# madsjulia/GeostatInversion.jl

Measured on AMD Instinct MI355X. Metric: randSVD GB/s + top-k singular-value rel-err, n=1e6 rank=256, higher is better.
Workload: dtype f64

## Files before the change

### geostatinversion.jl_amd/_lib.py

```python
import ctypes as C
import os

import numpy as np

_HERE = os.path.dirname(os.path.abspath(__file__))
LIB_PATH = os.path.join(_HERE, "libgsi_hip.so")

GSI_OK = 0
ERR_NAMES = {1: "GSI_ERR_ARG", 2: "GSI_ERR_NEG_ITERS", 3: "GSI_ERR_SINGULAR", 4: "GSI_ERR_HIP",
             5: "GSI_ERR_RCCL", 6: "GSI_ERR_OOM", 7: "GSI_ERR_NOT_POSDEF", 8: "GSI_ERR_INTERNAL"}
PHASES = ["gemm_n", "gemm_t", "lu", "qr", "svd", "small_gemm", "comm", "other", "comm_wait"]
UNIQUE_ID_BYTES = 128

c_i64 = C.c_int64
c_dp = C.POINTER(C.c_double)
c_vp = C.c_void_p
RANDN_FN = C.CFUNCTYPE(None, c_vp, c_dp, c_i64)

SIGNATURES = {
    "gsi_version": (C.c_int, []),
    "gsi_last_error": (C.c_char_p, []),
    "gsi_backend_name": (C.c_char_p, []),
    "gsi_ctx_create": (C.c_int, [C.POINTER(c_vp), C.c_int]),
    "gsi_ctx_destroy": (C.c_int, [c_vp]),
    "gsi_ctx_sync": (C.c_int, [c_vp]),
    "gsi_comm_unique_id": (C.c_int, [c_vp]),
    "gsi_ctx_comm_init": (C.c_int, [c_vp, C.c_int, C.c_int, c_vp]),
    "gsi_ctx_rank": (C.c_int, [c_vp, C.POINTER(C.c_int), C.POINTER(C.c_int)]),
    "gsi_ctx_host_allgather": (C.c_int, [c_vp, c_dp, c_i64, c_dp]),
    "gsi_op_dense": (C.c_int, [c_vp, C.POINTER(c_vp), c_dp, c_i64, c_i64, c_i64, c_i64, c_i64]),
    "gsi_op_lowrank": (C.c_int, [c_vp, C.POINTER(c_vp), c_dp, c_i64, c_i64, c_i64, C.c_int, c_i64, c_i64]),
    "gsi_op_lowrank_synthetic": (C.c_int, [c_vp, C.POINTER(c_vp), c_i64, c_i64, C.c_uint64, C.c_double, c_i64, c_i64]),
    "gsi_op_lowrank_samples": (C.c_int, [c_vp, c_vp, c_dp, c_i64]),
    "gsi_fftrf_fields": (C.c_int, [c_vp, c_vp, C.c_int, C.POINTER(c_i64), C.c_double, C.c_double, C.c_double, c_dp, c_i64,
                                   C.c_uint64, c_i64]),
    "gsi_op_lowrank_fftrf": (C.c_int, [c_vp, C.POINTER(c_vp), C.c_int, C.POINTER(c_i64), C.c_double, C.c_double, C.c_double,
                                       c_i64, C.c_uint64, c_i64, c_i64]),
    "gsi_fftrf_interpolate": (C.c_int, [c_vp, c_vp, c_vp, C.c_int, C.POINTER(c_i64), c_dp, c_i64, c_dp, c_i64]),
    "gsi_fftrf_spread": (C.c_int, [c_vp, c_vp, c_vp, C.c_int, C.POINTER(c_i64), c_dp, c_i64, c_dp, c_i64]),
    "gsi_fftrf_fields_at": (C.c_int, [c_vp, c_vp, C.c_int, C.POINTER(c_i64), C.c_double, C.c_double, C.c_double, c_dp, c_i64,
                                      C.c_uint64, c_i64, c_dp, c_i64, c_dp, c_i64]),
    "gsi_op_lowrank_fftrf_at": (C.c_int, [c_vp, C.POINTER(c_vp), C.c_int, C.POINTER(c_i64), C.c_double, C.c_double, C.c_double,
                                          c_i64, C.c_uint64, c_dp, c_i64, c_dp, c_i64, c_i64]),
    "gsi_op_dense_gridcov": (C.c_int, [c_vp, C.POINTER(c_vp), c_i64, c_i64, C.c_double, C.c_int, c_i64, c_i64]),
    "gsi_op_gridcov_implicit": (C.c_int, [c_vp, C.POINTER(c_vp), c_i64, c_i64, C.c_double, c_i64, c_i64]),
    "gsi_op_gridcov_implicit_kind": (C.c_int, [c_vp, C.POINTER(c_vp), c_i64, c_i64, C.c_double, C.c_int, c_i64, c_i64]),
    "gsi_op_gridcov_implicit_table": (C.c_int, [c_vp, C.POINTER(c_vp), c_i64, c_i64, c_dp, c_i64, c_i64]),
    "gsi_op_pointcov_implicit": (C.c_int, [c_vp, C.POINTER(c_vp), c_dp, c_i64, C.c_int, C.c_int, C.c_double, C.c_double,
                                           C.c_double, c_i64, c_i64]),
    "gsi_op_fft_powerlaw": (C.c_int, [c_vp, C.POINTER(c_vp), C.c_int, C.POINTER(c_i64), C.c_double]),
    "gsi_op_fft_powerlaw_fftrf": (C.c_int, [c_vp, C.POINTER(c_vp), C.c_int, C.POINTER(c_i64), C.c_double]),
    "gsi_op_fft_gridcov": (C.c_int, [c_vp, C.POINTER(c_vp), C.c_int, C.POINTER(c_i64), C.c_int, c_dp, C.c_double, C.c_double,
                                     C.c_double]),
    "gsi_op_fft_gridcov_table": (C.c_int, [c_vp, C.POINTER(c_vp), C.c_int, C.POINTER(c_i64), c_dp, c_dp, C.c_double]),
    "gsi_op_fft_at": (C.c_int, [c_vp, C.POINTER(c_vp), c_vp, c_dp, c_i64, c_dp]),
    "gsi_gridcov_sampler_create": (C.c_int, [c_vp, C.POINTER(c_vp), C.c_int, C.POINTER(c_i64), C.POINTER(c_i64), C.c_int, c_dp,
                                             C.c_double, C.c_double, C.c_double, C.c_double, c_dp]),
    "gsi_gridcov_sampler_info": (C.c_int, [c_vp, C.POINTER(c_i64), c_dp]),
    "gsi_gridcov_sampler_spectrum": (C.c_int, [c_vp, c_vp, c_dp]),
    "gsi_gridcov_sampler_destroy": (C.c_int, [c_vp]),
    "gsi_gridcov_fields": (C.c_int, [c_vp, c_vp, c_vp, c_dp, c_i64, C.c_uint64, c_i64]),
    "gsi_op_lowrank_gridcov": (C.c_int, [c_vp, C.POINTER(c_vp), c_vp, c_i64, C.c_uint64, c_i64, c_i64]),
    "gsi_op_destroy": (C.c_int, [c_vp]),
    "gsi_op_size": (C.c_int, [c_vp, C.POINTER(c_i64), C.POINTER(c_i64), C.POINTER(c_i64), C.POINTER(c_i64)]),
    "gsi_op_mul": (C.c_int, [c_vp, c_vp, C.c_int, c_dp, c_i64, c_i64, c_dp, c_i64]),
    "gsi_rangefinder": (C.c_int, [c_vp, c_vp, c_dp, c_i64, c_i64, c_dp]),
    "gsi_randsvd": (C.c_int, [c_vp, c_vp, c_dp, c_i64, c_i64, c_i64, c_dp, c_dp]),
    "gsi_randsvd_dense_host": (C.c_int, [c_vp, c_dp, c_i64, c_i64, c_i64, c_dp, c_i64, c_i64, c_i64, c_dp, c_dp, C.POINTER(c_vp)]),
    "gsi_rangefinder_dense_host": (C.c_int, [c_vp, c_dp, c_i64, c_i64, c_i64, c_dp, c_i64, c_i64, c_dp, C.POINTER(c_vp)]),
    "gsi_eig_nystrom": (C.c_int, [c_vp, c_vp, c_dp, c_i64, c_dp, c_dp]),
    "gsi_rangefinder_adaptive": (C.c_int, [c_vp, c_vp, RANDN_FN, c_vp, C.c_double, c_i64, c_dp, C.POINTER(c_i64)]),
    "gsi_mat_create": (C.c_int, [c_vp, C.POINTER(c_vp), c_i64, c_i64]),
    "gsi_mat_destroy": (C.c_int, [c_vp]),
    "gsi_mat_upload": (C.c_int, [c_vp, c_vp, c_dp, c_i64]),
    "gsi_mat_download": (C.c_int, [c_vp, c_vp, c_dp, c_i64]),
    "gsi_mat_randn": (C.c_int, [c_vp, c_vp, C.c_uint64]),
    "gsi_op_mul_dev": (C.c_int, [c_vp, c_vp, C.c_int, c_vp, c_vp]),
    "gsi_rangefinder_dev": (C.c_int, [c_vp, c_vp, c_vp, c_i64, c_vp]),
    "gsi_randsvd_dev": (C.c_int, [c_vp, c_vp, c_vp, c_i64, c_i64, c_i64, c_vp, c_vp]),
    "gsi_randsvd_rows": (C.c_int, [c_vp, c_vp, c_vp, c_i64, c_i64, c_i64, c_vp, c_vp]),
    "gsi_lu_L": (C.c_int, [c_vp, c_dp, c_i64, c_i64, c_dp, C.POINTER(C.c_int32)]),
    "gsi_lu_L_dev": (C.c_int, [c_vp, c_vp, C.POINTER(C.c_int32)]),
    "gsi_lu_L_sharded": (C.c_int, [c_vp, c_dp, c_i64, c_i64, c_dp, C.POINTER(C.c_int32)]),
    "gsi_lu_L_sharded_virtual": (C.c_int, [c_vp, c_dp, c_i64, c_i64, C.c_int, c_dp, C.POINTER(C.c_int32)]),
    "gsi_qr_thinQ": (C.c_int, [c_vp, c_dp, c_i64, c_i64, c_dp, c_dp]),
    "gsi_svd_tall": (C.c_int, [c_vp, c_dp, c_i64, c_i64, c_dp, c_dp]),
    "gsi_gemm": (C.c_int, [c_vp, C.c_int, c_i64, c_i64, c_i64, C.c_double, c_dp, c_i64, c_dp, c_i64, c_dp, c_i64]),
    "gsi_gemm_view": (C.c_int, [c_vp, C.c_int, C.c_int, c_i64, c_i64, c_i64, C.c_double, C.c_double, c_dp, c_i64, c_i64,
                                c_dp, c_i64, c_i64, c_dp, c_i64, c_i64, c_i64, c_i64, C.POINTER(c_i64)]),
    "gsi_cq_gram_round": (C.c_int, [c_vp, c_i64, C.c_int, c_dp, c_dp, c_dp, C.POINTER(C.c_int32), C.POINTER(C.c_int32),
                                    C.POINTER(C.c_double)]),
    "gsi_pcga_params": (C.c_int, [c_vp, c_dp, c_i64, c_i64, c_dp, c_dp, C.c_double, c_dp]),
    "gsi_pcga_update": (C.c_int, [c_vp, c_dp, c_i64, c_i64, c_dp, C.c_double, c_dp, c_i64, c_dp, c_dp]),
    "gsi_pcga_params_dev": (C.c_int, [c_vp, c_vp, c_i64, c_dp, c_dp, C.c_double, c_dp]),
    "gsi_pcga_update_dev": (C.c_int, [c_vp, c_vp, c_i64, c_dp, C.c_double, c_dp, c_i64, c_dp, c_dp]),
    "gsi_mat_download_col": (C.c_int, [c_vp, c_vp, c_i64, c_dp]),
    "gsi_op_lowrank_solve": (C.c_int, [c_vp, c_vp, c_dp, c_dp, C.POINTER(c_i64)]),
    "gsi_op_solve_cg": (C.c_int, [c_vp, c_vp, c_dp, c_vp, c_vp, C.c_double, c_i64, C.POINTER(c_i64), c_dp, C.POINTER(c_i64)]),
    "gsi_op_solve": (C.c_int, [c_vp, c_vp, c_dp, c_dp, c_i64, c_i64, c_dp, c_i64, C.c_double, c_i64, C.POINTER(c_i64), c_dp,
                               C.POINTER(c_i64)]),
    "gsi_mat_axpy": (C.c_int, [c_vp, C.c_double, c_vp, c_vp]),
    "gsi_precond_lowrank_create": (C.c_int, [c_vp, C.POINTER(c_vp), c_vp, c_i64, c_dp, C.c_double, c_dp]),
    "gsi_precond_destroy": (C.c_int, [c_vp]),
    "gsi_precond_info": (C.c_int, [c_vp, c_dp]),
    "gsi_precond_apply": (C.c_int, [c_vp, c_vp, c_vp, c_vp]),
    "gsi_op_solve_pcg": (C.c_int, [c_vp, c_vp, c_dp, c_vp, c_vp, c_vp, C.c_double, c_i64, C.POINTER(c_i64), c_dp,
                                   C.POINTER(c_i64)]),
    "gsi_op_solve_pcg_host": (C.c_int, [c_vp, c_vp, c_dp, c_vp, c_dp, c_i64, c_i64, c_dp, c_i64, C.c_double, c_i64,
                                        C.POINTER(c_i64), c_dp, C.POINTER(c_i64)]),
    "gsi_op_solve_trace": (C.c_int, [c_vp, c_vp, c_dp, c_vp, c_vp, c_vp, c_i64, c_i64, C.c_double, c_i64, C.POINTER(c_i64), c_dp,
                                     C.POINTER(c_i64), c_dp]),
    "gsi_slq_quadrature": (C.c_int, [c_vp, c_dp, c_dp, C.POINTER(c_i64), c_dp, c_i64, c_i64, c_dp]),
    "gsi_precond_sample": (C.c_int, [c_vp, c_vp, c_vp, c_vp, c_vp]),
    "gsi_precond_logdet": (C.c_int, [c_vp, c_dp]),
    "gsi_op_pivoted_cholesky": (C.c_int, [c_vp, c_vp, c_i64, C.c_double, c_vp, C.POINTER(c_i64), C.POINTER(c_i64), c_dp]),
    "gsi_mat_principal_factor": (C.c_int, [c_vp, c_vp, c_i64, c_vp, c_dp]),
    "gsi_pcgamat_create": (C.c_int, [c_vp, C.POINTER(c_vp), c_dp, c_i64, c_i64, c_dp, c_dp, C.c_int]),
    "gsi_pcgamat_destroy": (C.c_int, [c_vp]),
    "gsi_pcgamat_mul": (C.c_int, [c_vp, c_vp, c_dp, c_dp]),
    "gsi_pcgamat_lsqr": (C.c_int, [c_vp, c_vp, c_dp, c_dp, C.POINTER(c_i64)]),
    "gsi_pcgamat_solve": (C.c_int, [c_vp, c_vp, c_dp, c_dp, C.POINTER(c_i64)]),
    "gsi_chol_lower": (C.c_int, [c_vp, c_dp, c_i64, c_i64, c_dp, C.POINTER(c_i64)]),
    "gsi_basis_create": (C.c_int, [c_vp, C.POINTER(c_vp), c_vp, c_i64, C.c_int]),
    "gsi_basis_destroy": (C.c_int, [c_vp]),
    "gsi_pcga_params_basis": (C.c_int, [c_vp, c_vp, c_dp, c_dp, C.c_double, c_dp]),
    "gsi_pcga_update_basis": (C.c_int, [c_vp, c_vp, c_dp, C.c_double, c_dp, c_i64, c_dp, c_dp]),
    "gsi_basis_download_col": (C.c_int, [c_vp, c_vp, c_i64, c_dp]),
    "gsi_fwd_linear_create": (C.c_int, [c_vp, C.POINTER(c_vp), c_i64, c_i64, C.POINTER(c_i64), C.POINTER(c_i64), c_dp, c_dp,
                                        C.c_int]),
    "gsi_fwd_destroy": (C.c_int, [c_vp]),
    "gsi_fwd_info": (C.c_int, [c_vp, C.POINTER(c_i64), c_i64]),
    "gsi_fwd_apply": (C.c_int, [c_vp, c_vp, c_dp, c_i64, c_i64, c_dp, c_i64]),
    "gsi_fwd_apply_dev": (C.c_int, [c_vp, c_vp, c_vp, c_vp]),
    "gsi_fwd_adjoint_dev": (C.c_int, [c_vp, c_vp, c_vp, c_vp]),
    "gsi_fwd_adjoint_info": (C.c_int, [c_vp, C.POINTER(c_i64), c_i64]),
    "gsi_op_fwd_cov": (C.c_int, [c_vp, C.POINTER(c_vp), c_vp, c_vp]),
    "gsi_pcga_forward_basis": (C.c_int, [c_vp, c_vp, c_vp, c_dp, c_dp, C.c_double, c_dp]),
    "gsi_basis_quadform": (C.c_int, [c_vp, c_vp, c_dp, c_i64, c_i64, C.c_int, c_dp, c_dp, c_dp, c_dp, C.POINTER(c_i64)]),
    "gsi_pcgamat_posterior": (C.c_int, [c_vp, c_vp, c_dp, c_dp, c_dp, C.POINTER(c_i64)]),
    "gsi_pcga_posterior_variance": (C.c_int, [c_vp, c_vp, c_vp, c_dp, c_dp, c_dp, C.POINTER(c_i64)]),
    "gsi_op_posterior_variance": (C.c_int, [c_vp, c_vp, c_dp, c_dp, c_i64, c_i64, c_i64, c_dp, C.POINTER(c_i64)]),
    "gsi_mat_rowdot_acc": (C.c_int, [c_vp, c_vp, c_vp, c_vp]),
    "gsi_ctx_profile": (C.c_int, [c_vp, C.c_int]),
    "gsi_ctx_phase_reset": (C.c_int, [c_vp]),
    "gsi_ctx_phase_times": (C.c_int, [c_vp, c_dp, C.POINTER(c_i64)]),
    "gsi_ctx_counters": (C.c_int, [c_vp, C.POINTER(c_i64)]),
    "gsi_ctx_path_info": (C.c_int, [c_vp, C.POINTER(c_i64), c_i64]),
    "gsi_ctx_pinned_copy_rate": (C.c_int, [c_vp, c_i64, c_dp, c_dp]),
    "gsi_ctx_release_cache": (C.c_int, [c_vp]),
    "gsi_ctx_device_bytes": (C.c_int, [c_vp, C.POINTER(c_i64)]),
}


class GsiError(RuntimeError):

    def __init__(self, code, msg):
        super().__init__(f"{ERR_NAMES.get(code, code)}: {msg}")
        self.code = code


_lib = None


def load(path=None):
    global _lib
    if _lib is not None and path is None:
        return _lib
    p = path or os.environ.get("GSI_HIP_LIB") or LIB_PATH
    if not os.path.exists(p):
        raise ImportError(
            f"{p} not found: build it with `python {os.path.join(_HERE, 'build.py')}` (needs hipcc). "
            "This package has no CPU fallback.")
    lib = C.CDLL(p, mode=C.RTLD_LOCAL)
    for name, (res, args) in SIGNATURES.items():
        fn = getattr(lib, name)
        fn.restype = res
        fn.argtypes = args
    if path is None:
        _lib = lib
    return lib


def check(status, lib=None):
    if status != GSI_OK:
        lib = lib or load()
        raise GsiError(status, (lib.gsi_last_error() or b"").decode("utf-8", "replace"))


def fmat(a, name="matrix"):
    arr = np.asarray(a, dtype=np.float64)
    if arr.ndim == 1:
        arr = arr.reshape(-1, 1)
    if arr.ndim != 2:
        raise ValueError(f"{name} must be 1-D or 2-D")
    return np.asfortranarray(arr)


def dptr(arr):
    return arr.ctypes.data_as(c_dp)
```

### geostatinversion.jl_amd/build.py

```python
import os
import shutil
import subprocess
import sys
from concurrent.futures import ThreadPoolExecutor

HERE = os.path.dirname(os.path.abspath(__file__))
CSRC = os.path.join(HERE, "csrc")
OBJ = os.path.join(HERE, "build")
LIB = os.path.join(HERE, "libgsi_hip.so")
SOURCES = ["gemm_f64.hip", "gemm_f64_gen1.hip", "syrk_f64.hip", "panel_lu_leaf.hip", "panel_lu_blocks.hip", "panel_lu_streamed.hip", "panel_lu_sharded.hip", "panel_qr.hip", "cholqr.hip", "lowrank_power.hip", "jacobi_svd.hip", "misc.hip", "lsqr_dev.hip", "block_cg.hip", "block_pcg.hip", "block_slq.hip", "pivoted_chol.hip", "pointcov_gemm.hip", "fft_cov.hip", "fft_gridcov_plan.hip", "fftrf_sample.hip", "fftrf_interp.hip", "interp_adjoint.hip", "gridcov_sample.hip","pcga_forward.hip", "fwd_adjoint.hip", "chol_saddle.hip", "posterior_var.hip", "posterior_exact.hip",
           "hip_backend.hip", "hip_backend_products.hip", "hip_backend_sampler.hip", "hip_backend_panels.hip", "hip_backend_lowrank.hip", "hip_backend_pcga.hip",
           "hip_comm.hip", "pipeline.cpp", "solvers.cpp", "pcga.cpp", "api.cpp"]
HEADERS = ["backend.hpp", "hip_backend.hpp", "hip_backend_impl.hpp", "hip_common.hpp", "panel_lu_dev.hpp", "pipeline.hpp", "solvers.hpp", "pcga.hpp", "lsqr_state.hpp", "cg_state.hpp", "block_cg_host.hpp", "slq_state.hpp", "pchol_state.hpp", "pivoted_chol_host.hpp", "pointcov.hpp", "pointcov_gen.hpp", "host_staging.hpp", "gemm_f64_kernel.inc.hpp", "fft_line.hpp", "jacobi_sched.hpp", "fwd_plan.hpp", "fwd_adjoint_plan.hpp", "fwd_adjoint_host.hpp", "fftrf_points.hpp", "interp_adjoint_plan.hpp", "saddle_host.hpp", "posterior_host.hpp", "posterior_exact_host.hpp", "../../include/gsi_hip.h"]
CXXFLAGS = ["-O3", "-std=c++17", "-fPIC", "--offload-arch=gfx950", "-Wall", "-Wno-unused-function",
            "-Wno-unused-result", "-Wno-unused-value"]
RESOURCE_FLAG = "-Rpass-analysis=kernel-resource-usage"
_RES_KEYS = {"TotalSGPRs": "sgprs", "VGPRs": "vgprs", "AGPRs": "agprs", "ScratchSize [bytes/lane]": "scratch_bytes_per_lane",
             "Occupancy [waves/SIMD]": "occupancy_waves_per_simd", "SGPRs Spill": "sgpr_spills", "VGPRs Spill": "vgpr_spills",
             "LDS Size [bytes/block]": "lds_bytes_per_block", "Dynamic Stack": "dynamic_stack"}


def parse_resource_remarks(text):
    out, cur = {}, None
    for line in text.splitlines():
        if "remark:" not in line or "[-Rpass-analysis=kernel-resource-usage]" not in line:
            continue
        body = line.split("remark:", 1)[1].replace("[-Rpass-analysis=kernel-resource-usage]", "").strip()
        if ":" not in body:
            continue
        key, val = [x.strip() for x in body.rsplit(":", 1)]
        if key == "Function Name":
            cur = out.setdefault(val, {})
        elif cur is not None and key in _RES_KEYS:
            cur[_RES_KEYS[key]] = (val == "True") if key == "Dynamic Stack" else int(val)
    return out


def hipcc_version():
    r = subprocess.run([_hipcc(), "--version"], capture_output=True, text=True)
    lines = [ln.strip() for ln in r.stdout.splitlines() if ln.strip()]
    return "; ".join(lines[:2])


def kernel_resources():
    import json
    res = {}
    for src in SOURCES:
        if not src.endswith(".hip"):
            continue
        path = os.path.join(OBJ, src.replace(".", "_") + ".resources.json")
        if not os.path.exists(path):
            raise RuntimeError(f"{path} missing: run build() (it recompiles sources whose resource record is absent)")
        for name, r in json.load(open(path)).items():
            res[name] = dict(r, source=src)
    return res


def _hipcc():
    for cand in (shutil.which("hipcc"), "/opt/rocm/bin/hipcc"):
        if cand and os.path.exists(cand):
            return cand
    raise RuntimeError("hipcc not found: libgsi_hip.so cannot be built (there is no CPU fallback)")


def _newer(target, deps):
    if not os.path.exists(target):
        return True
    t = os.path.getmtime(target)
    return any(os.path.getmtime(d) > t for d in deps)


def build(force=False, verbose=False):
    hipcc = _hipcc()
    os.makedirs(OBJ, exist_ok=True)
    hdrs = [os.path.join(CSRC, h) for h in HEADERS] + [os.path.abspath(__file__)]
    jobs = []
    objs = []
    for src in SOURCES:
        s = os.path.join(CSRC, src)
        o = os.path.join(OBJ, src.replace(".", "_") + ".o")
        objs.append(o)
        is_hip = src.endswith(".hip")
        resj = os.path.join(OBJ, src.replace(".", "_") + ".resources.json")
        if force or _newer(o, [s] + hdrs) or (is_hip and not os.path.exists(resj)):
            cmd = [hipcc] + CXXFLAGS + (["-x", "hip", RESOURCE_FLAG] if is_hip else []) + ["-c", s, "-o", o]
            jobs.append(cmd)

    def run(cmd):
        import json
        if verbose:
            print(" ".join(cmd), flush=True)
        r = subprocess.run(cmd, capture_output=True, text=True)
        if r.returncode != 0:
            raise RuntimeError("compile failed: %s\n%s\n%s" % (" ".join(cmd), r.stdout, r.stderr))
        if RESOURCE_FLAG in cmd:
            obj = cmd[cmd.index("-o") + 1]
            with open(obj[:-2] + ".resources.json", "w") as f:
                json.dump(parse_resource_remarks(r.stderr), f, indent=0, sort_keys=True)
            return "\n".join(ln for ln in r.stderr.splitlines() if "kernel-resource-usage" not in ln and not ln.startswith(" ") and "remark" not in ln)
        return r.stderr

    if jobs:
        with ThreadPoolExecutor(max_workers=min(6, len(jobs))) as ex:
            for warn in ex.map(run, jobs):
                if verbose and warn:
                    print(warn)
    if jobs or force or _newer(LIB, objs):
        run([hipcc, "-shared", "-fPIC", "--offload-arch=gfx950", "-Wl,-Bsymbolic", "-o", LIB] + objs + ["-ldl"])
    vfile = os.path.join(OBJ, "hipcc_version.txt")
    if jobs or force or not os.path.exists(vfile):
        with open(vfile, "w") as f:
            f.write(hipcc_version() + "\n")
    return LIB


if __name__ == "__main__":
    print(build(force="--force" in sys.argv, verbose=True))
```

### geostatinversion.jl_amd/csrc/api.cpp

```cpp
#include <cmath>
#include <cstdlib>
#include <cstring>
#include <memory>
#include <new>
#include <string>
#include <vector>
#include "../../include/gsi_hip.h"
#include "pcga.hpp"
#include "solvers.hpp"
#include "pointcov.hpp"
#include "fftrf_points.hpp"
#include "cg_state.hpp"

using namespace gsi;

struct gsi_ctx {
  Context c;
};
struct gsi_op {
  Operator op;
};
struct gsi_mat {
  gsi_ctx* ctx;
  Buf buf;
  int64_t rows, cols;
  int refs = 1;
};
static void mat_unref(gsi_mat* m) {
  if (m && --m->refs <= 0) delete m;
}
struct gsi_pcgamat {
  gsi_ctx* ctx;
  PcgaLowRank A;
};
struct gsi_precond {
  gsi_ctx* ctx;
  LowRankPrecond pc;
};
struct gsi_basis {
  gsi_ctx* ctx;
  int64_t n, K;
  int precision;
  const double* Z64;
  Buf buf32;
  gsi_mat* owner = nullptr;
  BasisRef ref() const { return BasisRef{precision == 32 ? (const void*)buf32.p : (const void*)Z64, precision, n, K}; }
};

struct gsi_fwd {
  gsi_ctx* ctx;
  std::shared_ptr<FwdModel> shared = std::make_shared<FwdModel>();
  FwdModel& m = *shared;
};

struct gsi_sampler {
  gsi_ctx* ctx;
  void* plan = nullptr;
  int ndims;
  int64_t N[3], M[3], n, Mtot;
  double info[4];
  ~gsi_sampler() { if (plan) ctx->c.be->gridcov_sampler_destroy(plan); }
};

namespace {
thread_local std::string g_last_error;

int fail(int code, const std::string& msg) {
  g_last_error = msg;
  return code;
}

template <class F>
int guarded(F&& f) {
  try {
    f();
    return GSI_OK;
  } catch (const Error& e) {
    return fail(e.code, e.what());
  } catch (const std::bad_alloc&) {
    return fail(GSI_ERR_OOM, "host allocation failed");
  } catch (const std::exception& e) {
    return fail(GSI_ERR_INTERNAL, e.what());
  } catch (...) {
    return fail(GSI_ERR_INTERNAL, "unknown error");
  }
}

template <class F>
int with_info(int64_t* info_out, F&& f) {
  PathInfo info;
  const int st = guarded([&] { f(info); });
  if (info_out) { info_out[0] = info.column; info_out[1] = info.path; }
  return st;
}

template <class F>
void with_retry(Context& c, F&& f) {
  try {
    f();
  } catch (const Error&) {
    if (!c.be->retryable_failure() || c.comm || getenv("GSI_NO_RETRY") != nullptr) throw;
    c.lu_timeouts_recovered += 1;
    f();
  }
}

#define REQUIRE(cond, msg) \
  do { if (!(cond)) throw Error(GSI_ERR_ARG, msg); } while (0)

void check_shard(Context& c, int64_t m, int64_t row0, int64_t mloc) {
  REQUIRE(row0 >= 0 && mloc >= 0 && row0 + mloc <= m, "row shard out of range");
  if (c.nranks() == 1) {
    REQUIRE(row0 == 0 && mloc == m, "single-rank context: the operator must hold all rows");
  } else {
    int64_t r0, ml;
    default_shard(m, c.nranks(), c.rank(), &r0, &ml);
    REQUIRE(r0 == row0 && ml == mloc,
            "multi-rank operators use the block-row layout: pad = ceil(m/nranks), row0 = rank*pad");
  }
}
}

extern "C" {

int gsi_version(void) { return GSI_VERSION; }
const char* gsi_last_error(void) { return g_last_error.c_str(); }
const char* gsi_backend_name(void) { return backend_name(); }

int gsi_ctx_create(gsi_ctx** ctx, int device_id) {
  return guarded([&] {
    REQUIRE(ctx != nullptr, "ctx is NULL");
    *ctx = nullptr;
    gsi_ctx* c = new gsi_ctx();
    try {
      c->c.be.reset(make_backend(device_id));
    } catch (...) {
      delete c;
      throw;
    }
    *ctx = c;
  });
}

int gsi_ctx_destroy(gsi_ctx* ctx) {
  return guarded([&] {
    if (!ctx) return;
    ctx->c.comm.reset();
    ctx->c.be.reset();
    delete ctx;
  });
}

int gsi_ctx_sync(gsi_ctx* ctx) {
  return guarded([&] {
    REQUIRE(ctx, "ctx is NULL");
    ctx->c.be->sync();
  });
}

int gsi_comm_unique_id(void* id_out) {
  return guarded([&] {
    REQUIRE(id_out, "id_out is NULL");
    comm_unique_id(id_out);
  });
}
// ... 768 lines not shown
    REQUIRE(ctx && op && randn && Q_out && ncols_out, "NULL argument");
    REQUIRE(op->op.ctx == &ctx->c, "operator belongs to another context");
    *ncols_out = rangefinder_adaptive(op->op, randn, user, epsilon, r, Q_out);
    check_async_errors(ctx->c);
  });
}

int gsi_mat_create(gsi_ctx* ctx, gsi_mat** mat, int64_t rows, int64_t cols) {
  return guarded([&] {
    REQUIRE(ctx && mat, "NULL argument");
    *mat = nullptr;
    REQUIRE(rows >= 1 && cols >= 1, "bad shape");
    std::unique_ptr<gsi_mat> m(new gsi_mat());
    m->ctx = ctx; m->rows = rows; m->cols = cols;
    m->buf = Buf(ctx->c.be.get(), (size_t)rows * cols);
    *mat = m.release();
  });
}
int gsi_mat_destroy(gsi_mat* mat) {
  return guarded([&] { mat_unref(mat); });
}
int gsi_mat_upload(gsi_ctx* ctx, gsi_mat* mat, const double* host, int64_t ldh) {
  return guarded([&] {
    REQUIRE(ctx && mat && host && mat->ctx == ctx, "bad argument");
    REQUIRE(ldh >= mat->rows, "leading dimension too small");
    ctx->c.be->upload2d(mat->buf.p, mat->rows, host, ldh, mat->rows, mat->cols);
  });
}
int gsi_mat_download(gsi_ctx* ctx, const gsi_mat* mat, double* host, int64_t ldh) {
  return guarded([&] {
    REQUIRE(ctx && mat && host && mat->ctx == ctx, "bad argument");
    REQUIRE(ldh >= mat->rows, "leading dimension too small");
    ctx->c.be->download2d(host, ldh, mat->buf.p, mat->rows, mat->rows, mat->cols);
  });
}
int gsi_mat_randn(gsi_ctx* ctx, gsi_mat* mat, uint64_t seed) {
  return guarded([&] {
    REQUIRE(ctx && mat && mat->ctx == ctx, "bad argument");
    ctx->c.be->randn(mat->buf.p, (size_t)mat->rows * mat->cols, seed);
  });
}

int gsi_op_mul_dev(gsi_ctx* ctx, const gsi_op* op, int trans, const gsi_mat* X, gsi_mat* Y) {
  return guarded([&] {
    REQUIRE(ctx && op && X && Y, "NULL argument");
    REQUIRE(op->op.ctx == &ctx->c && X->ctx == ctx && Y->ctx == ctx, "objects belong to another context");
    const Operator& A = op->op;
    const int64_t l = X->cols;
    const int64_t rows_in = trans ? A.m : A.n, rows_out = trans ? A.n : A.m;
    REQUIRE(X->rows == rows_in && Y->rows == rows_out && Y->cols == l, "shape mismatch");
    if (!trans) {
      if (ctx->c.nranks() == 1) {
        op_mul(A, X->buf.p, A.n, l, Y->buf.p, A.m);
      } else {
        Buf Yloc(ctx->c.be.get(), (size_t)(A.mloc > 0 ? A.mloc : 1) * l);
        op_mul(A, X->buf.p, A.n, l, Yloc.p, A.mloc);
        gather_rows(ctx->c, A, Yloc.p, A.mloc, l, Y->buf.p);
      }
    } else {
      op_mul_t(A, X->buf.p + A.row0, A.m, l, Y->buf.p, A.n);
    }
  });
}

int gsi_rangefinder_dev(gsi_ctx* ctx, const gsi_op* op, const gsi_mat* Omega, int64_t numiterations,
                        gsi_mat* Q) {
  return guarded([&] {
    REQUIRE(ctx && op && Omega && Q, "NULL argument");
    REQUIRE(op->op.ctx == &ctx->c && Omega->ctx == ctx && Q->ctx == ctx, "objects belong to another context");
    const Operator& A = op->op;
    const int64_t l = Omega->cols;
    REQUIRE(Omega->rows == A.n, "Omega must have size(A,2) rows");
    REQUIRE(Q->rows == A.m && Q->cols == l, "Q must be size(A,1) x l");
    with_retry(ctx->c, [&] {
      Buf Qloc = rangefinder(A, Omega->buf.p, l, numiterations);
      gather_rows(ctx->c, A, Qloc.p, A.mloc, l, Q->buf.p);
      check_async_errors(ctx->c);
    });
  });
}

int gsi_randsvd_dev(gsi_ctx* ctx, const gsi_op* op, const gsi_mat* Omega, int64_t K, int64_t p, int64_t q,
                    gsi_mat* Z, gsi_mat* S) {
  return guarded([&] {
    REQUIRE(ctx && op && Omega && Z, "NULL argument");
    REQUIRE(op->op.ctx == &ctx->c && Omega->ctx == ctx && Z->ctx == ctx, "objects belong to another context");
    REQUIRE(K >= 0 && p >= 0 && K + p >= 1, "need K >= 0, p >= 0, K + p >= 1");
    const Operator& A = op->op;
    const int64_t l = K + p;
    REQUIRE(Omega->rows == A.n && Omega->cols == l, "Omega must be size(A,2) x (K+p)");
    REQUIRE(Z->rows == A.n && Z->cols == l, "Z must be size(A,2) x (K+p)");
    Backend* be = ctx->c.be.get();
    Buf Stmp;
    double* Sp;
    if (S) {
      REQUIRE(S->ctx == ctx && S->rows * S->cols == l, "S must hold K+p values");
      Sp = S->buf.p;
    } else {
      Stmp = Buf(be, (size_t)l);
      Sp = Stmp.p;
    }
    with_retry(ctx->c, [&] {
      randsvd(A, Omega->buf.p, K, p, q, Z->buf.p, Sp);
      check_async_errors(ctx->c);
    });
  });
}

int gsi_randsvd_rows(gsi_ctx* ctx, const gsi_op* op, const gsi_mat* Omega_rows, int64_t K, int64_t p, int64_t q,
                     gsi_mat* Z_rows, gsi_mat* S) {
  return guarded([&] {
    REQUIRE(ctx && op && Omega_rows && Z_rows, "NULL argument");
    REQUIRE(op->op.ctx == &ctx->c && Omega_rows->ctx == ctx && Z_rows->ctx == ctx, "objects belong to another context");
    REQUIRE(K >= 0 && p >= 0 && K + p >= 1, "need K >= 0, p >= 0, K + p >= 1");
    const Operator& A = op->op;
    const int64_t l = K + p;
    int64_t r0, nloc;
    default_shard(A.n, ctx->c.nranks(), ctx->c.rank(), &r0, &nloc);
    REQUIRE(nloc >= 1, "this rank holds no rows of the panel");
    REQUIRE(Omega_rows->rows == nloc && Omega_rows->cols == l, "Omega_rows must be (this rank's rows of size(A,2)) x (K+p)");
    REQUIRE(Z_rows->rows == nloc && Z_rows->cols == l, "Z_rows must be (this rank's rows of size(A,2)) x (K+p)");
    Backend* be = ctx->c.be.get();
    Buf Stmp;
    double* Sp;
    if (S) {
      REQUIRE(S->ctx == ctx && S->rows * S->cols == l, "S must hold K+p values");
      Sp = S->buf.p;
    } else {
      Stmp = Buf(be, (size_t)l);
      Sp = Stmp.p;
    }
    with_retry(ctx->c, [&] {
      randsvd_rows(A, Omega_rows->buf.p, K, p, q, Z_rows->buf.p, Sp);
      check_async_errors(ctx->c);
    });
  });
}

int gsi_lu_L(gsi_ctx* ctx, const double* Y, int64_t m, int64_t l, double* L_out, int32_t* ipiv_out) {
  return guarded([&] {
    REQUIRE(ctx && Y && L_out, "NULL argument");
    REQUIRE(m >= 1 && l >= 1 && l <= m, "lu_L: need 1 <= l <= m (tall panel)");
    Backend* be = ctx->c.be.get();
    Buf P(be, (size_t)m * l);
    with_retry(ctx->c, [&] {
      be->upload2d(P.p, m, Y, m, m, l);
      be->lu_L(P.p, m, l, m, ipiv_out);
      check_async_errors(ctx->c);
    });
    be->download2d(L_out, m, P.p, m, m, l);
  });
}

int gsi_lu_L_dev(gsi_ctx* ctx, gsi_mat* Y, int32_t* ipiv_out) {
  return guarded([&] {
    REQUIRE(ctx && Y, "NULL argument");
    REQUIRE(Y->ctx == ctx, "matrix belongs to another context");
    REQUIRE(Y->rows >= 1 && Y->cols >= 1 && Y->cols <= Y->rows, "lu_L: need 1 <= l <= m (tall panel)");
    Backend* be = ctx->c.be.get();
    {
      ScopedPhase ph(be, PH_LU);
      be->lu_L(Y->buf.p, Y->rows, Y->cols, Y->rows, ipiv_out);
    }
    check_async_errors(ctx->c);
  });
}

int gsi_lu_L_sharded(gsi_ctx* ctx, const double* Y, int64_t m, int64_t l, double* L_out, int32_t* ipiv_out) {
  return guarded([&] {
    REQUIRE(ctx && Y && L_out, "NULL argument");
    REQUIRE(m >= 1 && l >= 1 && l <= m, "lu_L: need 1 <= l <= m (tall panel)");
    Context& c = ctx->c;
    Backend* be = c.be.get();
    int64_t r0, ml;
    default_shard(m, c.nranks(), c.rank(), &r0, &ml);
    int64_t r00, ml0;
    default_shard(m, c.nranks(), 0, &r00, &ml0);
    REQUIRE(l <= ml0, "sharded lu: the first rank must hold the first l rows (l <= ceil(m / nranks))");
    Buf P(be, (size_t)std::max<int64_t>(ml, 1) * l);
    if (ml > 0) be->upload2d(P.p, ml, Y + r0, m, ml, l);
    lu_panel_sharded(c, P.p, m, r0, ml, l);
    Buf Full(be, (size_t)m * l);
    Operator shape;
    shape.m = m; shape.row0 = r0; shape.mloc = ml;
    gather_rows(c, shape, P.p, std::max<int64_t>(ml, 1), l, Full.p);
    be->download2d(L_out, m, Full.p, m, m, l);
    if (ipiv_out) be->lus_pivots(ipiv_out, l);
    check_async_errors(c);
  });
}

int gsi_lu_L_sharded_virtual(gsi_ctx* ctx, const double* Y, int64_t m, int64_t l, int nshards, double* L_out,
                             int32_t* ipiv_out) {
  return guarded([&] {
    REQUIRE(ctx && Y && L_out, "NULL argument");
    REQUIRE(m >= 1 && l >= 1 && l <= m, "lu_L: need 1 <= l <= m (tall panel)");
    REQUIRE(nshards >= 1 && nshards <= 64, "need 1 <= nshards <= 64");
    REQUIRE(nshards == 1 || l <= (m + nshards - 1) / nshards,
            "sharded lu: the first shard must hold the first l rows (l <= ceil(m / nshards))");
    Context& c = ctx->c;
    Backend* be = c.be.get();
    std::vector<Buf> shards;
    std::vector<double*> ptrs;
    for (int g = 0; g < nshards; ++g) {
      int64_t r0, ml;
      default_shard(m, nshards, g, &r0, &ml);
      shards.emplace_back(be, (size_t)std::max<int64_t>(ml, 1) * l);
      if (ml > 0) be->upload2d(shards.back().p, ml, Y + r0, m, ml, l);
      ptrs.push_back(shards.back().p);
    }
    lu_panel_sharded_virtual(c, ptrs.data(), m, l, nshards);
    check_async_errors(c);
    for (int g = 0; g < nshards; ++g) {
      int64_t r0, ml;
      default_shard(m, nshards, g, &r0, &ml);
      if (ml > 0) be->download2d(L_out + r0, m, ptrs[(size_t)g], ml, ml, l);
    }
    if (ipiv_out) be->lus_pivots(ipiv_out, l);
  });
}

int gsi_qr_thinQ(gsi_ctx* ctx, const double* Y, int64_t m, int64_t l, double* Q_out, double* R_out) {
  return guarded([&] {
    REQUIRE(ctx && Y && Q_out, "NULL argument");
    REQUIRE(m >= 1 && l >= 1 && l <= m, "qr_thinQ: need 1 <= l <= m (tall panel)");
    Backend* be = ctx->c.be.get();
    Buf P(be, (size_t)m * l), R(be, (size_t)l * l);
    be->upload2d(P.p, m, Y, m, m, l);
    {
      ScopedPhase ph(be, PH_QR);
      be->qr_thinQ(P.p, m, l, m, R.p);
    }
    be->download2d(Q_out, m, P.p, m, m, l);
    if (R_out) be->download2d(R_out, l, R.p, l, l, l);
    check_async_errors(ctx->c);
  });
}

int gsi_svd_tall(gsi_ctx* ctx, const double* W, int64_t n, int64_t l, double* V_out, double* S_out) {
  return guarded([&] {
    REQUIRE(ctx && W && V_out && S_out, "NULL argument");
    REQUIRE(n >= 1 && l >= 1 && l <= n, "svd_tall: need 1 <= l <= n");
    Backend* be = ctx->c.be.get();
    Buf Wd(be, (size_t)n * l), V(be, (size_t)n * l), S(be, (size_t)l);
    be->upload2d(Wd.p, n, W, n, n, l);
    svd_tall(ctx->c, Wd.p, n, l, -1, V.p, S.p);
    be->download2d(V_out, n, V.p, n, n, l);
    be->download2d(S_out, l, S.p, l, l, 1);
    check_async_errors(ctx->c);
  });
}

int gsi_gemm(gsi_ctx* ctx, int trans, int64_t m, int64_t l, int64_t k, double alpha, const double* A,
             int64_t lda, const double* B, int64_t ldb, double* C, int64_t ldc) {
  return guarded([&] {
    REQUIRE(ctx && A && B && C, "NULL argument");
    REQUIRE(m >= 1 && l >= 1 && k >= 1, "bad shape");
    const int64_t ar = trans ? k : m, ac = trans ? m : k;
    REQUIRE(lda >= ar && ldb >= k && ldc >= m, "leading dimension too small");
    Backend* be = ctx->c.be.get();
    Buf Ad(be, (size_t)ar * ac), Bd(be, (size_t)k * l), Cd(be, (size_t)m * l);
    be->upload2d(Ad.p, ar, A, lda, ar, ac);
    be->upload2d(Bd.p, k, B, ldb, k, l);
    if (trans) be->gemm_tn(m, l, k, alpha, Ad.p, ar, Bd.p, k, 0.0, Cd.p, m);
    else be->gemm_nn(m, l, k, alpha, Ad.p, ar, Bd.p, k, 0.0, Cd.p, m);
    be->download2d(C, ldc, Cd.p, m, m, l);
    check_async_errors(ctx->c);
  });
}

int gsi_gemm_view(gsi_ctx* ctx, int form, int trans, int64_t m, int64_t l, int64_t k, double alpha, double beta,
                  const double* A, int64_t lda, int64_t a_off, const double* B, int64_t ldb, int64_t b_off, double* C,
                  int64_t ldc, int64_t c_off, int64_t m_full, int64_t r0, int64_t* plan_out) {
  return guarded([&] {
    REQUIRE(ctx && A && C && plan_out, "NULL argument");
    REQUIRE(form >= 0 && form <= 3, "gemm_view: form is 0 (gemm), 1 (syrk upper), 2 (trmm upper) or 3 (NN row block)");
    REQUIRE(m >= 1 && l >= 1 && k >= 1, "bad shape");
    REQUIRE(form == 1 || B, "NULL argument");
    REQUIRE(form == 0 || (alpha == 1.0 && beta == 0.0), "gemm_view: forms 1 to 3 compute C = op(A) B (alpha 1, beta 0)");
    REQUIRE(form == 0 || !trans, "gemm_view: trans belongs to form 0");
    REQUIRE(form != 1 || m == l, "gemm_view: form 1 is the l x l product A'A (m == l)");
    REQUIRE(form != 3 || (r0 >= 0 && r0 + m <= m_full), "gemm_view: row block outside the full product");
    const bool tn = trans || form == 1;
    const int64_t ar = (form == 3) ? m_full : (tn ? k : m), ac = tn ? m : k;
    const int64_t crows = (form == 3) ? m_full : m;
    REQUIRE(lda >= ar && ldc >= crows && (form == 1 || ldb >= k), "leading dimension too small");
    REQUIRE(a_off >= 0 && b_off >= 0 && c_off >= 0, "negative offset");
    Backend* be = ctx->c.be.get();
    const size_t na = (size_t)a_off + (size_t)lda * (size_t)ac, nc = (size_t)c_off + (size_t)ldc * (size_t)l;
    const size_t nb = (form == 1) ? 1 : (size_t)b_off + (size_t)ldb * (size_t)l;
    Buf Ad(be, na), Bd(be, nb), Cd(be, nc);
    be->fill_bytes(Ad.p, 0xFF, na);
    be->fill_bytes(Bd.p, 0xFF, nb);
    be->upload2d(Ad.p + a_off, lda, A, ar, ar, ac);
    if (form != 1) be->upload2d(Bd.p + b_off, ldb, B, k, k, l);
    be->upload2d(Cd.p, (int64_t)nc, C, (int64_t)nc, (int64_t)nc, 1);
    be->gemm_view(form, trans != 0, m, l, k, alpha, Ad.p + a_off, lda, Bd.p + b_off, ldb, beta, Cd.p + c_off, ldc, m_full, r0,
                  plan_out);
    be->download2d(C, (int64_t)nc, Cd.p, (int64_t)nc, (int64_t)nc, 1);
    check_async_errors(ctx->c);
  });
}

int gsi_cq_gram_round(gsi_ctx* ctx, int64_t l, int check, const double* gram, double* R, double* X, int32_t* flag_out,
                      int32_t* series_out, double* norm_out) {
  return guarded([&] {
// ... 746 lines not shown
```

### geostatinversion.jl_amd/csrc/hip_backend_panels.hip

```cpp
#include <algorithm>
#include <cstdlib>
#include "hip_backend_impl.hpp"

namespace gsi {

void HipBackend::lu_L(double* Y, int64_t m, int64_t l, int64_t ld, int32_t* ipiv_host) {
  lu_L_impl(Y, m, l, ld, ipiv_host, nullptr);
}
bool HipBackend::lu_L_keep(double* Y, int64_t m, int64_t l, int64_t ld, int32_t** ipiv_dev) {
  if (ipiv_dev == nullptr) return false;
  lu_L_impl(Y, m, l, ld, nullptr, ipiv_dev);
  return true;
}
void HipBackend::lu_L_impl(double* Y, int64_t m, int64_t l, int64_t ld, int32_t* ipiv_host, int32_t** ipiv_dev_out) {
  bind();
  hipk::Lu2Work w2;
  static const int64_t ov_max = getenv("GSI_LU_OV_MAX") ? atoll(getenv("GSI_LU_OV_MAX")) : ((int64_t)5 << 20);
  static const bool ov_off = (getenv("GSI_LU_OV") != nullptr && getenv("GSI_LU_OV")[0] == '0');
  bool fits = lu2_takes(m, &w2);
  if (!fits && lu2_resident_ok() && !ov_off && m <= ov_max && ncus_ >= 1) {
    const int g = std::min(ncus_, 256);
    if (m > (int64_t)g * 4096) {
      if (lu2_ov_resident_ < 0) lu2_ov_resident_ = hipk::lu2_resident_per_cu_ov();
      if ((int64_t)lu2_ov_resident_ * ncus_ >= g) { w2.bs = 512; w2.rpt = 8; w2.grid = g; w2.ov = true; fits = true; }
    }
  }
  int32_t* ipiv_dev = nullptr;
  if (fits) {
    if (const char* e = getenv("GSI_LU_POLL_LIMIT")) w2.poll_limit = atoi(e);
    if (const char* e = getenv("GSI_LU_TEST_MUTE_EPOCH")) w2.mute_epoch = (uint32_t)atoi(e);
    if (const char* e = getenv("GSI_LU_COOPERATIVE")) w2.cooperative = (e[0] == '1');
    static const int nb_env = getenv("GSI_LU_NB") ? atoi(getenv("GSI_LU_NB")) : 0;
    w2.nb = (nb_env == 32 || nb_env == 64) ? nb_env : hipk::LU2_NB;
    grow(ws_lu_, hipk::lu2_work_bytes(l, w2.grid));
    hipk::lu2_carve(w2, l, ws_lu_.p);
    w2.info = flags_ + FLAG_LU_INFO;
    hipk::lu2_L(st_, Y, m, l, ld, w2);
    check_launch("lu2_L");
    ipiv_dev = w2.ipiv;
  } else {
    if (m >= ((int64_t)1 << 31)) throw Error(GSI_ERR_ARG, "lu: panels of 2^31 rows and more are not supported");
    grow(ws_lu_, hipk::lu3_work_bytes(l));
    hipk::lu3_L(st_, Y, m, l, ld, ws_lu_.p, flags_ + FLAG_LU_INFO, &ipiv_dev);
    check_launch("lu3_L");
  }
  if (ipiv_dev_out) *ipiv_dev_out = ipiv_dev;
  if (ipiv_host) {
    HIP_CHECK(hipMemcpyAsync(ipiv_host, ipiv_dev, sizeof(int32_t) * l, hipMemcpyDeviceToHost, st_));
    HIP_CHECK(hipStreamSynchronize(st_));
  }
}
bool HipBackend::lu2_resident_ok() const {
  static const bool tall_first = (getenv("GSI_LU_TALL") != nullptr && getenv("GSI_LU_TALL")[0] == '1');
  return !tall_first && !lu2_lost_ && ranks_sharing_device_ <= 1;
}
bool HipBackend::lu2_takes(int64_t m, hipk::Lu2Work* w) {
  return lu2_resident_ok() && hipk::lu2_config(m, ncus_, &w->bs, &w->rpt, &w->grid) && lu2_fits(w->bs, w->rpt, w->grid);
}
bool HipBackend::lu2_fits(int bs, int rpt, int grid) {
  const int key = bs * 16 + rpt;
  auto it = lu2_resident_.find(key);
  if (it == lu2_resident_.end()) it = lu2_resident_.emplace(key, hipk::lu2_resident_per_cu(bs, rpt)).first;
  return (int64_t)it->second * ncus_ >= grid;
}
struct HipBackend::LusWs { double* pval; int64_t* pidx; int32_t* ipiv; };
HipBackend::LusWs HipBackend::lus_ws(int64_t, int64_t l) {
  if (l > 8188) throw Error(GSI_ERR_ARG, "sharded lu: sketch width too large");
  Carve c;
  const size_t o_ipiv = c.take(32768), o_pval = c.take(sizeof(double) * 1024), o_pidx = c.take(sizeof(int64_t) * 1024);
  c.take(64);
  grow(ws_lus_, c.total);
  char* base = (char*)ws_lus_.p;
  LusWs w;
  w.ipiv = (int32_t*)(base + o_ipiv);
  w.pval = (double*)(base + o_pval);
  w.pidx = (int64_t*)(base + o_pidx);
  return w;
}
void HipBackend::lus_u12_leaf(const double* Yloc, int64_t ld, int64_t row0, int64_t jb, int64_t j0, int w, double* U12) {
  bind();
  hipk::lus_u12_leaf(st_, Yloc, ld, row0, jb, j0, w, U12);
  check_launch("lus_u12_leaf");
}
void HipBackend::lus_pending(double* Yloc, int64_t mloc, int64_t ld, int64_t row0, int64_t jb, int64_t j0, int w,
                             const double* U12) {
  bind();
  if (mloc > 0) hipk::lus_pending(st_, Yloc, ld, mloc, row0, jb, j0, w, U12);
  check_launch("lus_pending");
}
void HipBackend::lus_candidate(const double* Yloc, int64_t mloc, int64_t ld, int64_t row0, int64_t l, int64_t j, double* rec) {
  bind();
  LusWs w = lus_ws(mloc, l);
  const bool ready = (lus_part_col_ == j && lus_part_Y_ == Yloc && lus_part_mloc_ == mloc);
  lus_part_col_ = -1;
  hipk::lus_candidate(st_, Yloc, ld, mloc, row0, l, j, rec, w.pval, w.pidx, ready);
  check_launch("lus_candidate");
}
void HipBackend::lus_apply(double* Yloc, int64_t mloc, int64_t ld, int64_t row0, int64_t m, int64_t l, int64_t j0, int s, int w,
                           const double* recs, int nranks) {
  bind();
  LusWs ws = lus_ws(mloc, l);
  static const bool fuse = (getenv("GSI_LUS_NO_FUSE") == nullptr);
  const bool next = fuse && (s + 1 < w) && mloc > 0;
  hipk::lus_apply(st_, Yloc, ld, mloc, row0, m, l, j0, s, w, recs, nranks, ws.ipiv, flags_ + FLAG_LU_INFO, next ? ws.pval : nullptr,
                  next ? ws.pidx : nullptr);
  check_launch("lus_apply");
  lus_part_col_ = next ? j0 + s + 1 : -1;
  lus_part_Y_ = Yloc;
  lus_part_mloc_ = mloc;
}
void HipBackend::lus_u12_block(const double* Yloc, int64_t ld, int64_t row0, int64_t jb, int b, int64_t c0, int64_t c1,
                               double* U12) {
  bind();
  hipk::lus_u12_block(st_, Yloc, ld, row0, jb, b, c0, c1, U12);
  check_launch("lus_u12_block");
}
void HipBackend::lus_rankk(double* Yloc, int64_t mloc, int64_t ld, int64_t row0, int64_t jb, int b, int64_t c0, int64_t t,
                           const double* U12) {
  bind();
  hipk::lus_rankk(st_, Yloc, ld, mloc, row0, jb, b, c0, t, U12);
  check_launch("lus_rankk");
}
void HipBackend::lus_finish(double* Yloc, int64_t mloc, int64_t ld, int64_t row0, int64_t l) {
  bind();
  hipk::lus_finish(st_, Yloc, ld, mloc, row0, l);
}
bool HipBackend::lus_mr_begin(Comm* comm, int64_t m, int64_t l) {
  bind();
  auto no = [&](const std::string& why) { mr_reason_ = why; return false; };
  if (comm == nullptr) return no("no communicator");
  if (mr_comm_ != comm && !mr_share_tried_) {
    mr_share_tried_ = true;
    if (comm->nranks <= hipk::LU2_MAX_RANKS) {
      if (mr_recs_ == nullptr) {
        const size_t bytes = sizeof(unsigned long long) * hipk::lu2_mr_record_granules(1, 256);
        if (hipExtMallocWithFlags((void**)&mr_recs_, bytes, hipDeviceMallocFinegrained) != hipSuccess) {
          (void)hipGetLastError();
          HIP_CHECK(hipMalloc((void**)&mr_recs_, bytes));
        }
        HIP_CHECK(hipMemsetAsync(mr_recs_, 0, bytes, st_));
        HIP_CHECK(hipStreamSynchronize(st_));
        mr_epoch_ = 0;
      }
      void* all[hipk::LU2_MAX_RANKS] = {nullptr};
      if (comm->share_pointers(mr_recs_, 0, all)) {
        for (int g = 0; g < comm->nranks; ++g) mr_peer_[g] = (unsigned long long*)all[g];
        mr_comm_ = comm;
      } else {
        mr_disabled_ = true;
        mr_why_disabled_ = "the ranks' record buffers could not be mapped into each other (share_pointers)";
      }
    }
    lus_ws(1, 1);
  }
  static const bool off = (getenv("GSI_LU_NO_MR") != nullptr);
  if (off) return no("GSI_LU_NO_MR is set");
  if (mr_disabled_) return no("switched off on this context: " + mr_why_disabled_);
  if (mr_comm_ != comm) return no("another communicator owns this context's record buffers");
  if (comm->nranks > hipk::LU2_MAX_RANKS) return no("more than " + std::to_string(hipk::LU2_MAX_RANKS) + " ranks");
  if (m >= ((int64_t)1 << 28) || l > hipk::LU2_MR_MAXL) return no("panel too tall (2^28 rows) or too wide (" + std::to_string(hipk::LU2_MR_MAXL) + " columns)");
  const int G = comm->nranks;
  const int64_t pad = (m + G - 1) / G;
  hipk::Lu2MrWork w{};
  const int sharing = std::max(comm->ranks_on_my_device(), 1);
  const int se_cus = std::max(ncus_ / 32, 1);
  const int per_se = sharing > 1 ? std::max(se_cus / sharing, 0) : se_cus;
  if (per_se < 1)
    return no(std::to_string(sharing) + " ranks share this device, more than the " + std::to_string(se_cus) +
              " CUs of a shader engine: their persistent leaf grids cannot all be resident");
  if (!hipk::lu2_mr_config(pad, G, sharing > 1 ? per_se * 32 : ncus_, &w.bs, &w.rpt, &w.grid, &w.hier, &w.ov, mr_force_))
    return no("no launch geometry for shards of " + std::to_string(pad) + " rows on " + std::to_string(G) + " ranks (" +
              std::to_string(sharing) + " sharing this device)");
  const int key = 1000000 + w.bs * 16 + w.rpt + (w.ov ? 100000 : 0);
  auto it = lu2_resident_.find(key);
  if (it == lu2_resident_.end())
    it = lu2_resident_.emplace(key, w.ov ? hipk::lu2_mr_resident_per_cu_ov() : hipk::lu2_mr_resident_per_cu(w.bs, w.rpt)).first;
  if (sharing > 1 ? (int64_t)sharing * ((((w.grid + 7) / 8) + 3) / 4) > (int64_t)se_cus * it->second
                  : (int64_t)it->second * ncus_ < (int64_t)w.grid)
    return no("the leaf grids (" + std::to_string(w.grid) + " workgroups per rank, " + std::to_string(sharing) +
              " ranks on this device) would not all be resident");
  w.rank = comm->rank; w.nranks = G;
  for (int g = 0; g < G; ++g) w.peer[g] = mr_peer_[g];
  w.info = flags_ + FLAG_LU_INFO;
  if (const char* e = getenv("GSI_LU_POLL_LIMIT")) w.poll_limit = atoi(e);
  mr_work_ = w;
  mr_reason_.clear();
// ... 236 lines not shown
```

### geostatinversion.jl_amd/csrc/hip_common.hpp

```cpp
#pragma once
#include <hip/hip_runtime.h>
#include <atomic>
#include <cstdint>
#include <cstddef>
#include "pointcov.hpp"

namespace gsi { struct FwdProduct; struct FwdAdjoint; }

namespace gsi { namespace hipk {

inline bool first_use_on_this_device(std::atomic<uint64_t>& mask) {
  int dev = 0;
  if (hipGetDevice(&dev) != hipSuccess || dev < 0 || dev > 63) return true;
  const uint64_t bit = (uint64_t)1 << dev;
  return (mask.fetch_or(bit, std::memory_order_acq_rel) & bit) == 0;
}

struct GemmPlan { int64_t nt, nchunks, xmode, wide, nsplit, persistent, grid_x, active; };
size_t gemm_workspace_doubles(int64_t M, int64_t L, int64_t K);
void gemm_f64(hipStream_t st, bool transA, int64_t M, int64_t L, int64_t K, double alpha, const double* A,
              int64_t lda, const double* B, int64_t ldb, double beta, double* C, int64_t ldc, double* ws,
              GemmPlan* plan = nullptr);
bool gemm_f64_nn_capped(hipStream_t st, int64_t M, int64_t L, int64_t K, const double* A, int64_t lda, const double* B,
                        int64_t ldb, double* C, int64_t ldc, int max_grid, bool query_only = false, GemmPlan* plan = nullptr);
size_t gemm_rowblock_workspace_doubles(int64_t M_full, int64_t mb, int64_t L, int64_t K);
void gemm_f64_nn_rowblock(hipStream_t st, int64_t M_full, int64_t r0, int64_t mb, int64_t L, int64_t K, const double* A,
                          int64_t lda, const double* B, int64_t ldb, double* C, int64_t ldc, double* ws,
                          GemmPlan* plan = nullptr);
size_t gemm_syrk_workspace_doubles(int64_t l, int64_t m);
size_t syrk_upper_workspace_doubles(int64_t l, int64_t m);
bool syrk_full_from_upper(hipStream_t st, int64_t l, int64_t m, const double* Y, int64_t ld, double* G, int64_t ldg, double* ws);
bool trmm_upper_tall(hipStream_t st, int64_t m, int64_t l, const double* A, int64_t lda, const double* X, int64_t ldx, double* C,
                     int64_t ldc);
void gemm_f64_syrk_upper(hipStream_t st, int64_t l, int64_t m, const double* A, int64_t lda, double* C, int64_t ldc,
                         double* ws, GemmPlan* plan = nullptr);
void gemm_f64_trmm_upper(hipStream_t st, int64_t M, int64_t L, int64_t K, const double* A, int64_t lda, const double* B,
                         int64_t ldb, double* C, int64_t ldc, double* ws, GemmPlan* plan = nullptr);
void gemm_f64_gridcov(hipStream_t st, int64_t M, int64_t L, int64_t K, const double* tab, int64_t nx, int64_t ny,
                      int64_t roff, int64_t koff, const double* B, int64_t ldb, double* C, int64_t ldc, double* ws);

void gemm_f64_pointcov(hipStream_t st, int64_t M, int64_t L, int64_t K, const double* pts4, int64_t npts, int d, int kind,
                       double sigma2, double nugget, int64_t roff, int64_t koff, const double* B, int64_t ldb, double* C,
                       int64_t ldc, double* ws, double* xpack);
double pointcov_point_scale(int kind, double inv_ell);
bool gemm_f64_pointcov_wide(hipStream_t st, int64_t M, int64_t L, int64_t K, const double* pts4, int64_t npts, int d, int kind,
                            double sigma2, double nugget, int64_t roff, int64_t koff, const double* B, int64_t ldb, double* C,
                            int64_t ldc, double* ws, double* xpack);
size_t gemm_pointcov_workspace_doubles(int64_t M, int64_t L, int64_t K);
size_t gemm_pointcov_pack_doubles(int64_t M, int64_t L, int64_t K);
int gemm_choose_split(int64_t nwg, int64_t K);
void gemm_splitk_reduce(hipStream_t st, int64_t M, int64_t L, int nsplit, const double* slabs, double* C, int64_t ldc);
void pointcov_pad_points(hipStream_t st, const double* pts, int d, int64_t n, double scale, double* out4);
int64_t fft_embed_size(int64_t N);
size_t fft_plan_doubles(const int64_t M[3]);
void fft_spectrum(hipStream_t st, double* lam, double* part64, const int64_t M[3], double beta, int fftrf);
void fft_cos_matrix(hipStream_t st, double* out, int64_t rows, int64_t cols, int64_t period, bool weighted);
void fft_lines_layout(hipStream_t st, const double* nat, double* out, const int64_t M[3]);
void fft_spectrum_natural(hipStream_t st, double* lam, const int64_t M[3], double beta, int fftrf);
void fft_finish_plan(hipStream_t st, double* lam, double* part64, const int64_t M[3]);
void fft_plan_twiddles(hipStream_t st, double* lam, const int64_t M[3]);
void fft_lag_table(hipStream_t st, double* cp, double* cm, const int64_t N[3], int kind, const double inv_ell[3], double cs,
                   double sn, double sigma2);
void fft_even_odd_split(hipStream_t st, double* cp, double* cm, int64_t total);
void fft_sin_matrix(hipStream_t st, double* out, int64_t rows, int64_t cols, int64_t period);
void fft_subtract(hipStream_t st, double* a, const double* b, int64_t total);
void fft_finish_plan_lags(hipStream_t st, double* lam, const int64_t M[3], double nugget);
void fft_cov_apply(hipStream_t st, const int64_t N[3], const int64_t M[3], const double* lam, double2* W, int nb_max,
                   int64_t l, const double* X, int64_t ldx, double* Y, int64_t ldy);

struct FftrfGeom { int d; int64_t A[3], L[3], P[3]; int blue[3]; int64_t Mtot, n; };
void fftrf_geometry(int ndims, const int64_t* N, FftrfGeom* g);
size_t fftrf_plan_doubles(const FftrfGeom& g);
size_t fftrf_field_doubles(const FftrfGeom& g);
void fftrf_plan(hipStream_t st, const FftrfGeom& g, double* plan);
void fftrf_sample(hipStream_t st, const FftrfGeom& g, const double* plan, double* ws, int64_t fs, int nb, double k0, double dk,
                  double beta, double* dst, int64_t ldd, int64_t row0, int64_t nloc);
int fftrf_tile_lines(int Ma, bool contiguous, int64_t nl0);
void fftrf_twiddles(hipStream_t st, double* twg);
struct GcsGeom { int d; int64_t N[3], M[3]; int64_t Mtot, n; };
constexpr int GCS_PARTS = 64;
size_t gcs_pair_doubles(const GcsGeom& g);
void gcs_lag_table(hipStream_t st, const GcsGeom& g, int kind, const double inv_ell[3], double cs, double sn, double sigma2,
                   double* amp);
void gcs_plan_transform(hipStream_t st, const GcsGeom& g, const double* twg, const double* amp, double* W, double* lam);
void gcs_plan_finish(hipStream_t st, const GcsGeom& g, double nugget, double* lam, double* amp, double* part);
void gcs_sample(hipStream_t st, const GcsGeom& g, const double* twg, const double* amp, double* ws, int64_t fs, int nb,
                double* dst, int64_t ldd, int64_t row0, int64_t nloc, int64_t ncols);
void fftrf_interp(hipStream_t st, int d, const int32_t* base, const double* frac, int64_t m, int64_t s1, int64_t s2,
                  const double* V, int64_t v_fs, int nb, double* dst, int64_t ldd);
struct IadjDev {
  int d;
  int64_t n, m, chunk, nlong, nchunk;
  const int64_t* nodeptr;
  const int32_t* point;
  const uint8_t* corner;
  const double* frac;
  const int32_t* long_node;
  const int64_t* long_chunk0;
  const int64_t* chunk_off;
  const int32_t* chunk_len;
};
void interp_adjoint(hipStream_t st, const IadjDev& p, const double* X, int64_t ldx, int64_t nf, double* G, int64_t ldg,
                    double* partial);

constexpr int LU2_LEAF = 8;
constexpr int LU2_NB = 64;
constexpr int LU2_RES_COPIES = 8;
constexpr int LU2_REC_GRANULES = 64;
struct Lu2Work {
  unsigned long long* recs;
  double* u12;
  int32_t* ipiv;
  int32_t* info;
  int bs, rpt, grid, nb;
  int poll_limit = 0;
  uint32_t mute_epoch = 0;
  bool cooperative = false;
  bool ov = false;
};
int lu2_resident_per_cu_ov();
int lu2_resident_per_cu(int bs, int rpt);
constexpr int LU2_MAX_RANKS = 16;
constexpr int LU2_MR_MAXL = 8192;
struct Lu2MrWork {
  unsigned long long* peer[LU2_MAX_RANKS];
  int32_t* ipiv;
  int32_t* info;
  int rank, nranks, bs, rpt, grid;
  int hier = 0;
  int ov = 0;
  int poll_limit = 0;
};
bool lu2_mr_config(int64_t pad, int nranks, int ncus, int* bs, int* rpt, int* grid, int* hier, int* ov, int force = 0);
int lu2_mr_resident_per_cu(int bs, int rpt);
int lu2_mr_resident_per_cu_ov();
size_t lu2_mr_record_granules(int nranks, int grid);
void lu2_leaf_mr(hipStream_t st, const Lu2MrWork& w, double* Y, int64_t ld, int64_t mloc, int64_t row0, int64_t m, int64_t l,
                 int64_t jb, int64_t j0, int wd, const double* us, uint32_t epoch_base);
void lus_swap_peer(hipStream_t st, const Lu2MrWork& w, double* Y, int64_t ld, int64_t mloc, int64_t row0, int64_t m, int64_t l,
                   int64_t j0, int wd, uint32_t epoch_base);
void lus_swap_pack(hipStream_t st, const double* Y, int64_t ld, int64_t mloc, int64_t row0, int64_t l, int64_t j0, int w,
                   const int32_t* ipiv, double* table);
void lus_swap_apply(hipStream_t st, double* Y, int64_t ld, int64_t mloc, int64_t row0, int64_t l, int64_t j0, int w,
                    const int32_t* ipiv, const double* table);
bool lu2_config(int64_t m, int ncus, int* bs, int* rpt, int* grid);
size_t lu2_work_bytes(int64_t l, int grid);
void lu2_carve(Lu2Work& w, int64_t l, void* work);
void lu2_L(hipStream_t st, double* Y, int64_t m, int64_t l, int64_t ld, const Lu2Work& w);

size_t lu3_work_bytes(int64_t l);
void lu3_L(hipStream_t st, double* Y, int64_t m, int64_t l, int64_t ld, void* work, int32_t* info, int32_t** ipiv_out);

int lus_grid(int64_t mloc);
void lus_candidate(hipStream_t st, const double* Y, int64_t ld, int64_t mloc, int64_t row0, int64_t l, int64_t j, double* rec,
                   double* pval, int64_t* pidx, bool partials_ready);
void lus_apply(hipStream_t st, double* Y, int64_t ld, int64_t mloc, int64_t row0, int64_t m, int64_t l, int64_t j0, int s, int w,
               const double* recs, int nranks, int32_t* ipiv, int32_t* info, double* next_pval, int64_t* next_pidx);
void lus_u12_leaf(hipStream_t st, const double* Y, int64_t ld, int64_t row0, int64_t jb, int64_t j0, int w, double* U12);
void lus_pending(hipStream_t st, double* Y, int64_t ld, int64_t mloc, int64_t row0, int64_t jb, int64_t j0, int w,
                 const double* U12);
void lus_u12_block(hipStream_t st, const double* Y, int64_t ld, int64_t row0, int64_t jb, int b, int64_t c0, int64_t c1,
                   double* U12);
void lus_rankk(hipStream_t st, double* Y, int64_t ld, int64_t mloc, int64_t row0, int64_t jb, int b, int64_t c0, int64_t t,
               const double* U12);
void lus_finish(hipStream_t st, double* Y, int64_t ld, int64_t mloc, int64_t row0, int64_t l);
void lu_flag_export(hipStream_t st, const int32_t* info, double* flag);
void lu_flag_import(hipStream_t st, int32_t* info, const double* flag);

size_t lsqr_work_doubles();
void lsqr_begin(hipStream_t st, int64_t n, const double* w, double* work);
void lsqr_step_u(hipStream_t st, int64_t m, const double* t, double* u, double* work);
void lsqr_step_v(hipStream_t st, int64_t n, const double* t, double* v, double* w, double* x, double* work);

constexpr int BLOCK_CG_PARTS = 128;
size_t block_cg_work_doubles(int64_t b);
void block_cg_begin(hipStream_t st, int64_t n, int64_t b, const double* B, double tol, int64_t maxiter, double* work);
void block_cg_step(hipStream_t st, int64_t n, int64_t b, const double* Q, const double* d, double* X, double* R, double* P,
                   double* work);
bool block_cg_vec(int64_t n, const void* a, const void* b2, const void* c, const void* d, const void* e);
void block_cg_pass_pq(hipStream_t st, bool vec, int64_t n, int64_t b, const double* P, const double* Q, const double* d,
                      const double* s, double* part);
void block_cg_pass_xr(hipStream_t st, bool vec, int64_t n, int64_t b, const double* P, const double* Q, const double* d,
                      double* X, double* R, const double* s, double* part);

size_t block_pcg_work_doubles(int64_t b);
void block_pcg_begin(hipStream_t st, int64_t n, int64_t b, const double* B, const double* e, const double* Y, double* P,
                     double tol, int64_t maxiter, double* work);
void block_pcg_step_xr(hipStream_t st, int64_t n, int64_t b, const double* Q, const double* d, double* X, double* R,
                       const double* P, double* work);
void block_pcg_step_p(hipStream_t st, int64_t n, int64_t b, const double* e, const double* R, const double* Y, double* P,
                      double* work);
void pcg_precond_rows(hipStream_t st, int64_t n, double* e, double* sqe);
void pcg_add_identity(hipStream_t st, double* C, int64_t K);

void slq_trace_begin(hipStream_t st, const double* state, double* tr, int64_t qmax);
void slq_trace_step(hipStream_t st, const double* state, double* tr, int64_t qmax);
void slq_quadrature(hipStream_t st, const double* alpha, const double* beta, const double* steps, const double* rho0,
                    int64_t qmax, int64_t b, double* work, double* out);
void slq_sample_rows(hipStream_t st, int64_t n, int64_t b, const double* e, const double* Y, const double* G2, double* Zout);

struct PcholCol {
  int form;
  const double* a;
  int64_t ld;
  int32_t ny;
  int dim, kind;
  double sigma2, nugget;
};
size_t pchol_work_doubles(int form, int64_t n, int64_t K);
double* pchol_points(double* work, int64_t n, int64_t K);
void pchol_begin(hipStream_t st, const PcholCol& a, int64_t n, int64_t K, double tol, const double* L, int64_t ldl, double* d,
                 double* work);
void pchol_step(hipStream_t st, const PcholCol& a, int64_t n, int64_t K, double* L, int64_t ldl, double* d, double* work);
void scale_cols(hipStream_t st, int64_t n, int64_t K, double* U, int64_t ldu, const double* S);

constexpr int QR_NB = 16;
struct QrWork {
  double* coef;
  double* part;
  double* tau;
  double* T;
  double* G;
  double* Vbuf;
  double* Wt;
  double* W2;
  double* Qo;
  int64_t maxblocks;
};
int64_t qr_max_blocks(int64_t m);
void qr_thinQ(hipStream_t st, double* Y, int64_t m, int64_t l, int64_t ld, double* R, const QrWork& w,
              double* gemm_ws);
constexpr int QR_AMAX_PARTS = 256;
void qr_absmax(hipStream_t st, const double* Y, int64_t m, int64_t l, int64_t ld, double* amax_ws);
int qr_prescale_exponent(double amax);
void qr_scale(hipStream_t st, double* A, int64_t rows, int64_t cols, int64_t ld, double s);

size_t cholqr_small_doubles(int64_t l);
void cholqr2_factor(hipStream_t st, const double* Y, int64_t m, int64_t l, int64_t ld, double* T, int64_t ldt,
                    double* small_ws, int32_t* flag, double* gemm_ws);
void cholqr2_apply(hipStream_t st, double* Y, int64_t m, int64_t l, int64_t ld, const double* T, int64_t ldt,
                   double* R, double* small_ws, double* gemm_ws);
void cholqr2_R(hipStream_t st, int64_t l, double* small_ws, double* R);
const double* cholqr2_X2(const double* small_ws, int64_t l);
void mirror_upper(hipStream_t st, double* G, int64_t l);
bool cq_gram_round(hipStream_t st, double* Gm, int64_t l, double* X, bool check, int32_t* flag, int32_t* series = nullptr,
                   double* tmp = nullptr);
void tri_product(hipStream_t st, const double* R2, const double* R1, int64_t l, double* R);
bool tri_inverse(hipStream_t st, const double* R, int64_t l, double* X);
void lr_gather_rows(hipStream_t st, const double* S, int64_t lds, int64_t N, const int64_t* src, const int64_t* sub,
                    int64_t nr, double* R, int64_t ldr);
void lr_check_rows(hipStream_t st, const double* E, int64_t lde, const double* L, int64_t ldl, const int64_t* rows,
                   int64_t nchk, int64_t l, double* part, int nparts);
void scholqr3_factor(hipStream_t st, const double* Y, int64_t m, int64_t l, int64_t ld, double* T, int64_t ldt,
                     double* S, int64_t lds, double* small_ws, int32_t* flag, double* gemm_ws);
void scholqr3_apply(hipStream_t st, double* Y, int64_t m, int64_t l, int64_t ld, const double* S, int64_t lds,
                    double* R, double* small_ws, double* gemm_ws);

void lr_compose(hipStream_t st, const int32_t* piv, const int32_t* info, int64_t n, int64_t l, int64_t nchk, int64_t o_chk,
                int64_t o_sm, int64_t ldr, int64_t* src, int64_t* sub, int64_t* chk, int32_t* verdict);
void lr_solve_u(hipStream_t st, const double* L, int64_t ldl, const double* Mp, int64_t l, double c, double* Ut);
void lr_solve_c(hipStream_t st, const double* Ut, int64_t l, const double* T, int64_t N, double c, double* C);
void lr_solve_u12(hipStream_t st, const double* L, int64_t ldl, const double* Mp, int64_t l1, int64_t l, double c, double* Ut11,
                  double* U12);
void lr_move_rows(hipStream_t st, double* X, int64_t ldx, int64_t nc, const int64_t* src, const int64_t* sub,
                  const int32_t* verdict, int64_t maxmv, double* tmp, int64_t ldt, int64_t nzero);
void lr_pivots(hipStream_t st, const int32_t* piv, int64_t cnt, int64_t add, int32_t* dst);
void lr_forget_zero_pivot(hipStream_t st, int32_t* info);
// ... 65 lines not shown
```

### geostatinversion.jl_amd/csrc/panel_lu_blocks.hip

```cpp
#include "panel_lu_dev.hpp"
#include <type_traits>

namespace gsi { namespace hipk {

template <int K>
__device__ inline void u12_stage_L11(double* L11, const double* __restrict__ Y, int64_t ld, int64_t jb, int64_t jbrow) {
#pragma unroll 8
  for (int e = threadIdx.x; e < K * K; e += 256) {
    const int r = e % K, c = e / K;
    L11[r * K + c] = Y[(jbrow + r) + (jb + c) * ld];
  }
}
template <int K>
__device__ inline void u12_solve(const double* L11, double (&x)[K]) {
#pragma unroll
  for (int r = 1; r < K; ++r) {
    double v = x[r];
#pragma unroll
    for (int p = 0; p < r; ++p) v -= L11[r * K + p] * x[p];
    x[r] = v;
  }
}

template <int K>
__global__ __launch_bounds__(256) void lu_u12_kernel(const double* __restrict__ Y, int64_t ld, int64_t jb, int64_t jbrow,
                                                     int64_t c0, int64_t c1, double* __restrict__ out) {
  __shared__ double L11[K * K];
  u12_stage_L11<K>(L11, Y, ld, jb, jbrow);
  __syncthreads();
  if (threadIdx.x >= 64) return;
  const int64_t c = c0 + (int64_t)blockIdx.x * 64 + threadIdx.x;
  if (c >= c1) return;
  double x[K];
  const double* col = Y + jbrow + c * ld;
#pragma unroll
  for (int r = 0; r < K; ++r) x[r] = col[r];
  u12_solve<K>(L11, x);
  double* o = out + (c - c0) * K;
#pragma unroll
  for (int r = 0; r < K; ++r) o[r] = x[r];
}

template <int K, int DEPTH, int RK_CHUNK>
__global__ __launch_bounds__(256) __attribute__((amdgpu_waves_per_eu(RK_CHUNK == 64 ? 3 : 2, RK_CHUNK == 64 ? 3 : 4))) void lu_rankk_kernel(double* __restrict__ Y, int64_t ld, int64_t m, int64_t r_begin,
                                                       int64_t jb, int64_t c0, int64_t t,
                                                       const double* __restrict__ U12) {
  typedef double double4_t __attribute__((ext_vector_type(4)));
  constexpr int KP = K + 2;
  extern __shared__ double us[];
  const int tid = threadIdx.x, lane = tid & 63, wave = tid >> 6;
  const int jl = lane & 15, kk = lane >> 4;
  const int64_t rb = r_begin + ((int64_t)blockIdx.x * 4 + wave) * 32;
  double fa[2][K / 4];
#pragma unroll
  for (int h = 0; h < 2; ++h) {
    const int64_t rrow = rb + 16 * h + jl;
#pragma unroll
    for (int s = 0; s < K / 4; ++s) fa[h][s] = (rrow < m) ? Y[rrow + (jb + 4 * s + kk) * ld] : 0.0;
  }
  for (int64_t cc0 = 0; cc0 < t; cc0 += RK_CHUNK) {
    const int tc = (int)((t - cc0 < RK_CHUNK) ? (t - cc0) : RK_CHUNK);
    __syncthreads();
    for (int e = tid; e < RK_CHUNK * K; e += 256) {
      const int k = e % K, c = e / K;
      us[c * KP + k] = (c < tc) ? U12[k + (cc0 + c) * K] : 0.0;
    }
    __syncthreads();
    if (rb >= m) continue;
    const int ntile = (tc + 15) / 16;
    double cin[2][4];
    auto load_tile = [&](int tt, double (&dst)[2][4]) {
#pragma unroll
      for (int h = 0; h < 2; ++h) {
        const int64_t rrow = rb + 16 * h + jl;
#pragma unroll
        for (int reg = 0; reg < 4; ++reg) {
          const int cl = 16 * tt + kk + 4 * reg;
          dst[h][reg] = (rrow < m && cl < tc) ? Y[rrow + (c0 + cc0 + cl) * ld] : 0.0;
        }
      }
    };
    load_tile(0, cin);
    double cin2[2][4];
    if (DEPTH == 2 && ntile > 1) load_tile(1, cin2);
    for (int tt = 0; tt < ntile; ++tt) {
      double4_t acc[2];
#pragma unroll
      for (int h = 0; h < 2; ++h) acc[h] = (double4_t){cin[h][0], cin[h][1], cin[h][2], cin[h][3]};
      if (DEPTH == 2) {
#pragma unroll
        for (int h = 0; h < 2; ++h)
#pragma unroll
          for (int reg = 0; reg < 4; ++reg) cin[h][reg] = cin2[h][reg];
        if (tt + 2 < ntile) load_tile(tt + 2, cin2);
      } else if (tt + 1 < ntile) load_tile(tt + 1, cin);
#pragma unroll
      for (int s = 0; s < K / 4; ++s) {
        const double fb = -us[(16 * tt + jl) * KP + 4 * s + kk];
#pragma unroll
        for (int h = 0; h < 2; ++h) acc[h] = __builtin_amdgcn_mfma_f64_16x16x4f64(fb, fa[h][s], acc[h], 0, 0, 0);
      }
#pragma unroll
      for (int h = 0; h < 2; ++h) {
        const int64_t rrow = rb + 16 * h + jl;
#pragma unroll
        for (int reg = 0; reg < 4; ++reg) {
          const int cl = 16 * tt + kk + 4 * reg;
          if (rrow < m && cl < tc) Y[rrow + (c0 + cc0 + cl) * ld] = acc[h][reg];
        }
      }
    }
  }
}

template <int K, int DEPTH, int CHUNK>
static void launch_rankk_v(hipStream_t st, unsigned grid, double* Y, int64_t ld, int64_t m, int64_t r_begin, int64_t jb,
                           int64_t c0, int64_t t, const double* U12) {
  constexpr size_t shmem = (size_t)CHUNK * (K + 2) * sizeof(double);
  static std::atomic<uint64_t> attr_mask{0};
  if (first_use_on_this_device(attr_mask))
    (void)hipFuncSetAttribute((const void*)lu_rankk_kernel<K, DEPTH, CHUNK>, hipFuncAttributeMaxDynamicSharedMemorySize, (int)shmem);
  hipLaunchKernelGGL((lu_rankk_kernel<K, DEPTH, CHUNK>), dim3(grid), dim3(256), shmem, st, Y, ld, m, r_begin, jb, c0, t, U12);
}
template <int K>
static void launch_rankk(hipStream_t st, unsigned grid, double* Y, int64_t ld, int64_t m, int64_t r_begin, int64_t jb,
                         int64_t c0, int64_t t, const double* U12) {
  static const int depth = getenv("GSI_LU_RK_DEPTH") ? atoi(getenv("GSI_LU_RK_DEPTH")) : 1;
  static const int chunk = getenv("GSI_LU_RK_CHUNK") ? atoi(getenv("GSI_LU_RK_CHUNK")) : 64;
  if (chunk == 64 && depth == 2) launch_rankk_v<K, 2, 64>(st, grid, Y, ld, m, r_begin, jb, c0, t, U12);
  else if (chunk == 64) launch_rankk_v<K, 1, 64>(st, grid, Y, ld, m, r_begin, jb, c0, t, U12);
  else if (depth == 2) launch_rankk_v<K, 2, 128>(st, grid, Y, ld, m, r_begin, jb, c0, t, U12);
  else launch_rankk_v<K, 1, 128>(st, grid, Y, ld, m, r_begin, jb, c0, t, U12);
}

constexpr int LL_WAVES = 12;
constexpr int LL_BS = 64 * LL_WAVES;
constexpr size_t LL_LDS = (size_t)4 * 64 * 66 * sizeof(double);
template <int NB>
constexpr int ll_group() { return (int)(LL_LDS / ((size_t)NB * (NB + 2) * sizeof(double))); }

__device__ __forceinline__ char* ll_advance(char* p, int64_t step) {
  p += step;
  asm volatile("" : "+s"(p));
  return p;
}

template <int NB, bool WIDE>
__global__ __launch_bounds__(LL_BS) void lu_leftlook_kernel(double* __restrict__ Y, int64_t ld, int64_t m, int64_t jb, int tc,
                                                            int ip0, int ip1, const double* __restrict__ U12, int64_t ldu) {
  typedef double double4_t __attribute__((ext_vector_type(4)));
  typedef typename std::conditional<WIDE, uint64_t, uint32_t>::type off_t;
  constexpr int KP = NB + 2, NT = NB / 16, NS = NB / 4;
  extern __shared__ double us[];
  const int tid = threadIdx.x, lane = tid & 63;
  const int wave = __builtin_amdgcn_readfirstlane(tid >> 6);
  const int jl = lane & 15, kk = lane >> 4;
  const int nbk = ip1 - ip0;
  for (int e = tid; e < nbk * NB * NB; e += LL_BS) {
    const int k = e % NB, c = (e / NB) % NB, q = e / (NB * NB);
    us[(q * NB + c) * KP + k] = (c < tc) ? -U12[(int64_t)(ip0 + q) * ldu + (jb + c) * NB + k] : 0.0;
  }
  __syncthreads();
  const int lb = jl * KP + kk;
  const int64_t nch = (m - jb + 15) / 16;
  const int64_t cs = ld * (int64_t)sizeof(double);
  for (int64_t ch = (int64_t)blockIdx.x * LL_WAVES + wave; ch < nch; ch += (int64_t)gridDim.x * LL_WAVES) {
    const int64_t rb = jb + ch * 16;
    const int64_t r = (rb + jl < m) ? rb + jl : m - 1;
    const off_t vo = (off_t)((r - rb) * (int64_t)sizeof(double) + kk * cs);
    auto at = [&](char* colp) -> double* { return reinterpret_cast<double*>(colp + vo); };
    char* const cbase = reinterpret_cast<char*>(Y + rb + jb * ld);
    double4_t acc[NT];
    {
      char* p = cbase;
#pragma unroll
      for (int tt = 0; tt < NT; ++tt)
#pragma unroll
        for (int reg = 0; reg < 4; ++reg) {
          acc[tt][reg] = (16 * tt + 4 * reg + kk < tc) ? *at(p) : 0.0;
          p = ll_advance(p, 4 * cs);
        }
    }
    double fa[NS], fn[NS];
    char* pf = reinterpret_cast<char*>(Y + rb + (int64_t)ip0 * NB * ld);
    auto load_frag = [&](double (&f)[NS]) {
#pragma unroll
      for (int s = 0; s < NS; ++s) {
        f[s] = *at(pf);
        pf = ll_advance(pf, 4 * cs);
      }
    };
    auto run = [&](const double (&f)[NS], int q) {
      const double* ub = us + (q - ip0) * NB * KP + lb;
#pragma unroll
      for (int s = 0; s < NS; ++s)
#pragma unroll
        for (int tt = 0; tt < NT; ++tt)
          acc[tt] = __builtin_amdgcn_mfma_f64_16x16x4f64(ub[16 * tt * KP + 4 * s], f[s], acc[tt], 0, 0, 0);
    };
    load_frag(fa);
    int q = ip0;
    for (; q + 1 < ip1; ++q) {
      load_frag(fn);
      run(fa, q);
#pragma unroll
      for (int s = 0; s < NS; ++s) fa[s] = fn[s];
    }
    run(fa, q);
    const bool live = rb + jl < m;
    char* p = cbase;
#pragma unroll
    for (int tt = 0; tt < NT; ++tt)
#pragma unroll
      for (int reg = 0; reg < 4; ++reg) {
        if (live && 16 * tt + 4 * reg + kk < tc) *at(p) = acc[tt][reg];
        p = ll_advance(p, 4 * cs);
      }
  }
}

template <int K>
__global__ __launch_bounds__(256) void lu_urows_kernel(const double* __restrict__ Y, int64_t ld, int64_t jb, int nprev,
                                                       int64_t c0, int64_t c1, const double* __restrict__ U12, int64_t ldu,
                                                       double* __restrict__ out) {
  typedef double double4_t __attribute__((ext_vector_type(4)));
  constexpr int TP = K + 1;
  __shared__ double L11[K * K];
  __shared__ double T[64 * TP];
  u12_stage_L11<K>(L11, Y, ld, jb, jb);
  const int tid = threadIdx.x, lane = tid & 63, wave = tid >> 6;
  const int jl = lane & 15, kk = lane >> 4;
  const int64_t cb = c0 + (int64_t)blockIdx.x * 64;
  if (wave < K / 16) {
    const int64_t row = jb + 16 * wave + jl;
    double4_t acc[4];
#pragma unroll
    for (int tt = 0; tt < 4; ++tt)
#pragma unroll
      for (int reg = 0; reg < 4; ++reg) {
        const int64_t c = cb + 16 * tt + kk + 4 * reg;
        acc[tt][reg] = (c < c1) ? Y[row + c * ld] : 0.0;
      }
    for (int q = 0; q < nprev; ++q) {
      const double* ub = U12 + (int64_t)q * ldu;
#pragma unroll
      for (int s = 0; s < K / 4; ++s) {
        const double fa = Y[row + ((int64_t)q * K + 4 * s + kk) * ld];
#pragma unroll
        for (int tt = 0; tt < 4; ++tt) {
          const int64_t c = cb + 16 * tt + jl;
          const double fb = (c < c1) ? -ub[c * K + 4 * s + kk] : 0.0;
          acc[tt] = __builtin_amdgcn_mfma_f64_16x16x4f64(fb, fa, acc[tt], 0, 0, 0);
        }
      }
    }
#pragma unroll
    for (int tt = 0; tt < 4; ++tt)
#pragma unroll
      for (int reg = 0; reg < 4; ++reg) T[(16 * tt + kk + 4 * reg) * TP + 16 * wave + jl] = acc[tt][reg];
  }
  __syncthreads();
  if (tid >= 64) return;
  const int64_t c = cb + tid;
  if (c >= c1) return;
  double x[K];
#pragma unroll
  for (int r = 0; r < K; ++r) x[r] = T[tid * TP + r];
  u12_solve<K>(L11, x);
  double* o = out + (c - c0) * K;
#pragma unroll
  for (int r = 0; r < K; ++r) o[r] = x[r];
}

template <int NB, bool WIDE>
static void launch_leftlook_v(hipStream_t st, unsigned grid, double* Y, int64_t ld, int64_t m, int64_t jb, int tc,
                              const double* U12, int64_t ldu) {
  static std::atomic<uint64_t> attr_mask{0};
  if (first_use_on_this_device(attr_mask))
    (void)hipFuncSetAttribute((const void*)lu_leftlook_kernel<NB, WIDE>, hipFuncAttributeMaxDynamicSharedMemorySize, (int)LL_LDS);
  const int nprev = (int)(jb / NB);
  for (int ip0 = 0; ip0 < nprev; ip0 += ll_group<NB>()) {
    const int ip1 = std::min(nprev, ip0 + ll_group<NB>());
    const size_t shmem = (size_t)(ip1 - ip0) * NB * (NB + 2) * sizeof(double);
    hipLaunchKernelGGL((lu_leftlook_kernel<NB, WIDE>), dim3(grid), dim3(LL_BS), shmem, st, Y, ld, m, jb, tc, ip0, ip1, U12, ldu);
  }
}
static void lu_ll_update(hipStream_t st, double* Y, int64_t ld, int64_t m, int64_t l, int64_t jb, int b, int nb,
                         const double* u12) {
  if (jb == 0 || m <= jb) return;
  int dev = 0, ncu = 0;
  (void)hipGetDevice(&dev);
  if (hipDeviceGetAttribute(&ncu, hipDeviceAttributeMultiprocessorCount, dev) != hipSuccess || ncu < 1) ncu = 256;
  const int64_t chunks = (m - jb + 15) / 16;
  const unsigned grid = (unsigned)std::min<int64_t>((chunks + LL_WAVES - 1) / LL_WAVES, ncu);
  const bool wide = (3 * ld + 32) * (int64_t)sizeof(double) >= ((int64_t)1 << 32);
  const int64_t ldu = (int64_t)nb * l;
  if (nb == 64) {
    if (wide) launch_leftlook_v<64, true>(st, grid, Y, ld, m, jb, b, u12, ldu);
    else launch_leftlook_v<64, false>(st, grid, Y, ld, m, jb, b, u12, ldu);
  } else {
    if (wide) launch_leftlook_v<32, true>(st, grid, Y, ld, m, jb, b, u12, ldu);
    else launch_leftlook_v<32, false>(st, grid, Y, ld, m, jb, b, u12, ldu);
  }
}
static void lu_ll_urows(hipStream_t st, const double* Y, int64_t ld, int64_t l, int64_t jb, int nb, double* u12) {
  const int64_t c0 = jb + nb, ldu = (int64_t)nb * l;
  if (c0 >= l) return;
  const unsigned gu = (unsigned)((l - c0 + 63) / 64);
  double* out = u12 + (jb / nb) * ldu + c0 * nb;
  if (nb == 64) {
    if (jb == 0) hipLaunchKernelGGL(lu_u12_kernel<64>, dim3(gu), dim3(256), 0, st, Y, ld, jb, jb, c0, l, out);
    else hipLaunchKernelGGL(lu_urows_kernel<64>, dim3(gu), dim3(256), 0, st, Y, ld, jb, (int)(jb / nb), c0, l, u12, ldu, out);
  } else {
    if (jb == 0) hipLaunchKernelGGL(lu_u12_kernel<32>, dim3(gu), dim3(256), 0, st, Y, ld, jb, jb, c0, l, out);
    else hipLaunchKernelGGL(lu_urows_kernel<32>, dim3(gu), dim3(256), 0, st, Y, ld, jb, (int)(jb / nb), c0, l, u12, ldu, out);
  }
}

__global__ void lu2_extract_L_kernel(double* __restrict__ Y, int64_t ld, int64_t l) {
  const int64_t total = l * l;
  for (int64_t e = (int64_t)blockIdx.x * blockDim.x + threadIdx.x; e < total; e += (int64_t)gridDim.x * blockDim.x) {
    const int64_t r = e % l, c = e / l;
    if (r == c) Y[r + c * ld] = 1.0;
    else if (r < c) Y[r + c * ld] = 0.0;
  }
}

void lu_blocks(hipStream_t st, double* Y, int64_t ld, int64_t m, int64_t l, int nb, double* u12, const LuLeafFn& leaf) {
  for (int64_t jb = 0; jb < l; jb += nb) {
    const int b = (int)((l - jb < nb) ? (l - jb) : nb);
    lu_ll_update(st, Y, ld, m, l, jb, b, nb, u12);
    for (int64_t j0 = jb; j0 < jb + b; j0 += LW) leaf(jb, b, j0, (int)((jb + b - j0 < LW) ? (jb + b - j0) : LW));
    lu_ll_urows(st, Y, ld, l, jb, nb, u12);
  }
  int eb = (int)((l * l + 255) / 256);
  if (eb > 1024) eb = 1024;
  hipLaunchKernelGGL(lu2_extract_L_kernel, dim3(eb), dim3(256), 0, st, Y, ld, l);
}

void lus_u12_block(hipStream_t st, const double* Y, int64_t ld, int64_t row0, int64_t jb, int b, int64_t c0, int64_t c1,
                   double* U12) {
  const unsigned gu = (unsigned)((c1 - c0 + 63) / 64);
  if (b == 64) hipLaunchKernelGGL(lu_u12_kernel<64>, dim3(gu), dim3(256), 0, st, Y, ld, jb, jb - row0, c0, c1, U12);
  else hipLaunchKernelGGL(lu_u12_kernel<32>, dim3(gu), dim3(256), 0, st, Y, ld, jb, jb - row0, c0, c1, U12);
}
void lus_rankk(hipStream_t st, double* Y, int64_t ld, int64_t mloc, int64_t row0, int64_t jb, int b, int64_t c0, int64_t t,
               const double* U12) {
  int64_t rbeg = c0 - row0;
  if (rbeg < 0) rbeg = 0;
  const int64_t mr = mloc - rbeg;
  if (mr <= 0) return;
  const unsigned gr = (unsigned)((mr + 127) / 128);
  if (b == 64) launch_rankk<64>(st, gr, Y, ld, mloc, rbeg, jb, c0, t, U12);
  else launch_rankk<32>(st, gr, Y, ld, mloc, rbeg, jb, c0, t, U12);
}

}}
```

### geostatinversion.jl_amd/csrc/panel_lu_dev.hpp

```cpp
#pragma once
#include "hip_common.hpp"
#include <algorithm>
#include <cstdlib>
#include <functional>

namespace gsi { namespace hipk {

namespace {

constexpr int LW = LU2_LEAF;
constexpr int KPMAX = LU2_NB - LW;
constexpr int LSP = KPMAX + 1;
constexpr int REC = LU2_REC_GRANULES;
constexpr int POLL_LIMIT = 4000000;

__device__ inline double readlane_d(double x, int srclane) {
  int lo = __double2loint(x), hi = __double2hiint(x);
  lo = __builtin_amdgcn_readlane(lo, srclane);
  hi = __builtin_amdgcn_readlane(hi, srclane);
  return __hiloint2double(hi, lo);
}
template <int CTRL, int ROW_MASK>
__device__ inline double dpp_fmax(double v) {
  const int lo = __builtin_amdgcn_update_dpp(0, __double2loint(v), CTRL, ROW_MASK, 0xf, false);
  const int hi = __builtin_amdgcn_update_dpp((int)0xbff00000, __double2hiint(v), CTRL, ROW_MASK, 0xf, false);
  return fmax(v, __hiloint2double(hi, lo));
}
template <int CTRL, int ROW_MASK>
__device__ inline uint32_t dpp_umin(uint32_t v) {
  const uint32_t o = (uint32_t)__builtin_amdgcn_update_dpp((int)0xFFFFFFFFu, (int)v, CTRL, ROW_MASK, 0xf, false);
  return o < v ? o : v;
}
__device__ inline void wave_argmax(double& v, int32_t& i) {
  double mx = v;
  mx = dpp_fmax<0x111, 0xf>(mx);
  mx = dpp_fmax<0x112, 0xf>(mx);
  mx = dpp_fmax<0x114, 0xf>(mx);
  mx = dpp_fmax<0x118, 0xf>(mx);
  mx = dpp_fmax<0x142, 0xa>(mx);
  mx = dpp_fmax<0x143, 0xc>(mx);
  mx = __hiloint2double(__builtin_amdgcn_readlane(__double2hiint(mx), 63), __builtin_amdgcn_readlane(__double2loint(mx), 63));
  uint32_t key = (v == mx) ? (uint32_t)i : 0xFFFFFFFFu;
  key = dpp_umin<0x111, 0xf>(key);
  key = dpp_umin<0x112, 0xf>(key);
  key = dpp_umin<0x114, 0xf>(key);
  key = dpp_umin<0x118, 0xf>(key);
  key = dpp_umin<0x142, 0xa>(key);
  key = dpp_umin<0x143, 0xc>(key);
  v = mx;
  i = (int32_t)__builtin_amdgcn_readlane((int)key, 63);
}

__device__ inline void wave_argmax8(double& v, int32_t& i) {
  double mx = v;
  mx = dpp_fmax<0x111, 0xf>(mx);
  mx = dpp_fmax<0x112, 0xf>(mx);
  mx = dpp_fmax<0x114, 0xf>(mx);
  mx = __hiloint2double(__builtin_amdgcn_readlane(__double2hiint(mx), 7), __builtin_amdgcn_readlane(__double2loint(mx), 7));
  uint32_t key = (v == mx) ? (uint32_t)i : 0xFFFFFFFFu;
  key = dpp_umin<0x111, 0xf>(key);
  key = dpp_umin<0x112, 0xf>(key);
  key = dpp_umin<0x114, 0xf>(key);
  v = mx;
  i = (int32_t)__builtin_amdgcn_readlane((int)key, 7);
}

template <bool MR>
__device__ inline unsigned long long poll_granule(const unsigned long long* p) {
  if constexpr (MR) return __hip_atomic_load(p, __ATOMIC_RELAXED, __HIP_MEMORY_SCOPE_SYSTEM);
  else return __hip_atomic_load(p, __ATOMIC_RELAXED, __HIP_MEMORY_SCOPE_AGENT);
}

__device__ inline void lu_timeout_note(int32_t* info, int phase, int slot, uint32_t epoch, int who) {
  if (atomicCAS(info + 2, 0, phase) == 0) { info[3] = slot; info[4] = (int32_t)epoch; info[5] = who; }
}

}

struct LuMrArgs {
  int rank, nranks;
  int hier;
  int slots;
  int32_t gbase, mtot;
  const double* us;
  unsigned long long* peer[LU2_MAX_RANKS];
};

using LuLeafFn = std::function<void(int64_t jb, int b, int64_t j0, int wd)>;
void lu_blocks(hipStream_t st, double* Y, int64_t ld, int64_t m, int64_t l, int nb, double* u12, const LuLeafFn& leaf);

}}
```

### geostatinversion.jl_amd/csrc/panel_lu_leaf.hip

```cpp
#include "panel_lu_dev.hpp"
#include <cstdio>

namespace gsi { namespace hipk {

namespace {
#ifdef GSI_LU_TRACE
__device__ unsigned long long g_lu_trace[4 * 8 * 8];
#define LU_STAMP(ph)                                                                                    \
  do {                                                                                                  \
    if (tid == 0 && kp == 0) {                                                                          \
      const int tw = (g == 0) ? 0 : (g == 1) ? 1 : (g == G / 2) ? 2 : (g == G - 1) ? 3 : -1;              \
      if (tw >= 0) g_lu_trace[(tw * 8 + s) * 8 + (ph)] = wall_clock64();                                   \
    }                                                                                                   \
  } while (0)
#else
#define LU_STAMP(ph) do { } while (0)
#endif
}

template <int BS, int R, bool MR, bool OV = false>
__global__ __launch_bounds__(BS) void lu_leaf_kernel(double* __restrict__ Y, int64_t ld, int32_t m, int32_t l,
                                                     int32_t jb, int32_t j0, int w, unsigned long long* __restrict__ recs,
                                                     uint32_t epoch_base, int32_t* __restrict__ ipiv,
                                                     int32_t* __restrict__ info, int onehop, int poll_limit,
// ... 641 lines not shown
  for (int k = 0; k < LW; ++k) {
    if (k < w) {
      char* cb = colbase(j0 + k);
#pragma unroll
      for (int rr = 0; rr < R; ++rr) {
        const int32_t i = row0 + rr * BS;
        if (i < m) *elem(cb, i) = a[rr][k];
      }
      if (isdiag && drow < m) *elem(cb, drow) = d[k];
    }
  }
}

bool lu2_config(int64_t m, int ncus, int* bs, int* rpt, int* grid) {
  if (ncus < 1) return false;
  if (ncus > 256) ncus = 256;
  static const int cfg[4][2] = {{256, 1}, {256, 4}, {512, 4}, {512, 8}};
  for (int c = 0; c < 4; ++c) {
    const int64_t per = (int64_t)cfg[c][0] * cfg[c][1];
    if (m <= (int64_t)ncus * per) { *bs = cfg[c][0]; *rpt = cfg[c][1]; *grid = (int)((m + per - 1) / per); return true; }
  }
  return false;
}

template <int BS, int R>
static void launch_leaf(hipStream_t st, int grid, double* Y, int64_t ld, int64_t m, int64_t l, int64_t jb, int64_t j0,
                        int w, const Lu2Work& wk, uint32_t epoch_base) {
  static const int onehop = getenv("GSI_LU_ONEHOP") ? atoi(getenv("GSI_LU_ONEHOP")) : 1;
  const int poll_limit = wk.poll_limit > 0 ? wk.poll_limit : POLL_LIMIT;
  LuMrArgs none{};
  if constexpr (BS == 512 && R == 8) {
    if (wk.ov) {
      hipLaunchKernelGGL((lu_leaf_kernel<512, 8, false, true>), dim3(grid), dim3(512), 0, st, Y, ld, (int32_t)m, (int32_t)l,
                         (int32_t)jb, (int32_t)j0, w, wk.recs, epoch_base, wk.ipiv, wk.info, 1, poll_limit, wk.mute_epoch, none);
      return;
    }
  }
  if (!wk.cooperative) {
    hipLaunchKernelGGL((lu_leaf_kernel<BS, R, false>), dim3(grid), dim3(BS), 0, st, Y, ld, (int32_t)m, (int32_t)l, (int32_t)jb,
                       (int32_t)j0, w, wk.recs, epoch_base, wk.ipiv, wk.info, onehop, poll_limit, wk.mute_epoch, none);
    return;
  }
  int32_t m32 = (int32_t)m, l32 = (int32_t)l, jb32 = (int32_t)jb, j032 = (int32_t)j0;
  int oh = onehop, pl = poll_limit;
  uint32_t eb = epoch_base, mute = wk.mute_epoch;
  unsigned long long* recs = wk.recs;
  int32_t* ipiv = wk.ipiv;
  int32_t* info = wk.info;
  void* args[] = {&Y, &ld, &m32, &l32, &jb32, &j032, &w, &recs, &eb, &ipiv, &info, &oh, &pl, &mute, &none};
  (void)hipLaunchCooperativeKernel((const void*)lu_leaf_kernel<BS, R, false>, dim3(grid), dim3(BS), args, 0, st);
}

static int leaf_resident_per_cu(const void* kernel, int bs) {
  int nblk = 0;
  if (hipOccupancyMaxActiveBlocksPerMultiprocessor(&nblk, kernel, bs, 0) != hipSuccess) {
    (void)hipGetLastError();
    return 0;
  }
  return nblk;
}
int lu2_resident_per_cu_ov() { return leaf_resident_per_cu((const void*)lu_leaf_kernel<512, 8, false, true>, 512); }
int lu2_resident_per_cu(int bs, int rpt) {
  if (bs == 256 && rpt == 1) return leaf_resident_per_cu((const void*)lu_leaf_kernel<256, 1, false>, 256);
  if (bs == 256) return leaf_resident_per_cu((const void*)lu_leaf_kernel<256, 4, false>, 256);
  if (rpt == 4) return leaf_resident_per_cu((const void*)lu_leaf_kernel<512, 4, false>, 512);
  return leaf_resident_per_cu((const void*)lu_leaf_kernel<512, 8, false>, 512);
}

bool lu2_mr_config(int64_t pad, int nranks, int ncus, int* bs, int* rpt, int* grid, int* hier, int* ov, int force) {
  *ov = 0;
  if (nranks < 1 || nranks > LU2_MAX_RANKS) return false;
  if (force == 2) {
    if (nranks < 2 || pad <= 2 * 4096 || ncus < 2) return false;
    *bs = 512; *rpt = 8; *grid = 2; *hier = 1; *ov = 1;
    return true;
  }
  static const int ov_cap = getenv("GSI_LU_MR_OV_GRID") ? atoi(getenv("GSI_LU_MR_OV_GRID")) : 0;
  static const int64_t ov_max = getenv("GSI_LU_OV_MAX") ? atoll(getenv("GSI_LU_OV_MAX")) : ((int64_t)5 << 20);
  if (ov_cap > 0 && nranks > 1 && pad > (int64_t)ov_cap * 4096 && ov_cap <= std::min(256 - nranks, ncus)) {
    *bs = 512; *rpt = 8; *grid = ov_cap; *hier = 1; *ov = 1;
    return true;
  }
  static const int cfg[4][2] = {{256, 1}, {256, 4}, {512, 4}, {512, 8}};
  static const char* he = getenv("GSI_LU_MR_HIER");
  const bool force_hier = (he != nullptr && he[0] == '1') || force == 1, no_hier = he != nullptr && he[0] == '0' && force != 1;
  const int gmax = std::min(256 / nranks, ncus);
  for (int c = 0; c < 4 && !force_hier; ++c) {
    const int64_t per = (int64_t)cfg[c][0] * cfg[c][1];
    const int64_t g = (pad + per - 1) / per;
    if (g <= gmax) { *bs = cfg[c][0]; *rpt = cfg[c][1]; *grid = (int)std::max<int64_t>(g, 1); *hier = 0; return true; }
  }
  const int gmax2 = std::min(256 - nranks, ncus);
  for (int c = 0; c < 4 && !no_hier && nranks > 1; ++c) {
    const int64_t per = (int64_t)cfg[c][0] * cfg[c][1];
    const int64_t g = (pad + per - 1) / per;
    if (g <= gmax2) { *bs = cfg[c][0]; *rpt = cfg[c][1]; *grid = (int)std::max<int64_t>(g, 1); *hier = 1; return true; }
  }
  if (!no_hier && nranks > 1 && gmax2 >= 1 && pad <= ov_max && !(getenv("GSI_LU_OV") != nullptr && getenv("GSI_LU_OV")[0] == '0')) {
    *bs = 512; *rpt = 8; *grid = gmax2; *hier = 1; *ov = 1;
    return true;
  }
  return false;
}
template <int BS, int R>
static void launch_leaf_mr_t(hipStream_t st, const Lu2MrWork& w, double* Y, int64_t ld, int64_t mloc, int64_t row0, int64_t m,
                             int64_t l, int64_t jb, int64_t j0, int wd, const double* us, uint32_t epoch_base) {
  LuMrArgs a{};
  a.rank = w.rank; a.nranks = w.nranks; a.gbase = (int32_t)row0; a.mtot = (int32_t)m; a.us = us;
  a.hier = w.hier; a.slots = w.hier ? w.grid + w.nranks : w.nranks * w.grid;
  for (int q = 0; q < w.nranks; ++q) a.peer[q] = w.peer[q];
  const int poll_limit = w.poll_limit > 0 ? w.poll_limit : POLL_LIMIT;
  if constexpr (BS == 512 && R == 8) {
    if (w.ov) {
      hipLaunchKernelGGL((lu_leaf_kernel<512, 8, true, true>), dim3(w.grid), dim3(512), 0, st, Y, ld, (int32_t)mloc, (int32_t)l,
                         (int32_t)jb, (int32_t)j0, wd, w.peer[w.rank], epoch_base, w.ipiv, w.info, 1, poll_limit, 0u, a);
      return;
    }
  }
  hipLaunchKernelGGL((lu_leaf_kernel<BS, R, true>), dim3(w.grid), dim3(BS), 0, st, Y, ld, (int32_t)mloc, (int32_t)l, (int32_t)jb,
                     (int32_t)j0, wd, w.peer[w.rank], epoch_base, w.ipiv, w.info, 1, poll_limit, 0u, a);
}
void lu2_leaf_mr(hipStream_t st, const Lu2MrWork& w, double* Y, int64_t ld, int64_t mloc, int64_t row0, int64_t m, int64_t l,
                 int64_t jb, int64_t j0, int wd, const double* us, uint32_t epoch_base) {
  if (w.bs == 256 && w.rpt == 1) launch_leaf_mr_t<256, 1>(st, w, Y, ld, mloc, row0, m, l, jb, j0, wd, us, epoch_base);
  else if (w.bs == 256) launch_leaf_mr_t<256, 4>(st, w, Y, ld, mloc, row0, m, l, jb, j0, wd, us, epoch_base);
  else if (w.rpt == 4) launch_leaf_mr_t<512, 4>(st, w, Y, ld, mloc, row0, m, l, jb, j0, wd, us, epoch_base);
  else launch_leaf_mr_t<512, 8>(st, w, Y, ld, mloc, row0, m, l, jb, j0, wd, us, epoch_base);
}
int lu2_mr_resident_per_cu_ov() { return leaf_resident_per_cu((const void*)lu_leaf_kernel<512, 8, true, true>, 512); }
int lu2_mr_resident_per_cu(int bs, int rpt) {
  if (bs == 256 && rpt == 1) return leaf_resident_per_cu((const void*)lu_leaf_kernel<256, 1, true>, 256);
  if (bs == 256) return leaf_resident_per_cu((const void*)lu_leaf_kernel<256, 4, true>, 256);
  if (rpt == 4) return leaf_resident_per_cu((const void*)lu_leaf_kernel<512, 4, true>, 512);
  return leaf_resident_per_cu((const void*)lu_leaf_kernel<512, 8, true>, 512);
}
size_t lu2_mr_record_granules(int nranks, int grid) {
  return (size_t)2 * (size_t)nranks * (size_t)grid * REC + (size_t)2 * (2 * KPMAX * LW) + (size_t)2 * ((size_t)2 * LW * 2 * LU2_MR_MAXL);
}

static size_t lu2_record_bytes(int grid) { return sizeof(unsigned long long) * 2 * ((size_t)grid + LU2_RES_COPIES) * REC; }
size_t lu2_work_bytes(int64_t l, int grid) {
  return lu2_record_bytes(grid) + sizeof(double) * (size_t)l * (size_t)l + sizeof(int32_t) * (size_t)(l + 4) + 256;
}
void lu2_carve(Lu2Work& w, int64_t l, void* work) {
  char* base = (char*)work;
  w.recs = (unsigned long long*)base; base += lu2_record_bytes(w.grid);
  w.u12 = (double*)base; base += sizeof(double) * (size_t)l * (size_t)l;
  w.ipiv = (int32_t*)base;
}

void lu2_L(hipStream_t st, double* Y, int64_t m, int64_t l, int64_t ld, const Lu2Work& w) {
  (void)hipMemsetAsync(w.recs, 0, lu2_record_bytes(w.grid), st);
  uint32_t epoch = 0;
  lu_blocks(st, Y, ld, m, l, w.nb, w.u12, [&](int64_t jb, int, int64_t j0, int wd) {
    if (w.bs == 256 && w.rpt == 1) launch_leaf<256, 1>(st, w.grid, Y, ld, m, l, jb, j0, wd, w, epoch);
    else if (w.bs == 256) launch_leaf<256, 4>(st, w.grid, Y, ld, m, l, jb, j0, wd, w, epoch);
    else if (w.rpt == 4) launch_leaf<512, 4>(st, w.grid, Y, ld, m, l, jb, j0, wd, w, epoch);
    else launch_leaf<512, 8>(st, w.grid, Y, ld, m, l, jb, j0, wd, w, epoch);
    epoch += (uint32_t)LW;
  });
#ifdef GSI_LU_TRACE
  if (const char* path = getenv("GSI_LU_TRACE")) {
    unsigned long long h[4 * 8 * 8];
    (void)hipStreamSynchronize(st);
    (void)hipMemcpyFromSymbol(h, HIP_SYMBOL(g_lu_trace), sizeof(h));
    if (FILE* f = fopen(path, "w")) {
      for (int tw = 0; tw < 4; ++tw)
        for (int s = 0; s < 8; ++s) {
          fprintf(f, "wg%d step%d", tw, s);
          for (int ph = 0; ph < 6; ++ph) fprintf(f, " %llu", h[(tw * 8 + s) * 8 + ph]);
          fprintf(f, "\n");
        }
      fclose(f);
    }
  }
#endif
}

}}
```

### geostatinversion.jl_amd/csrc/panel_lu_streamed.hip

```cpp
#include "panel_lu_dev.hpp"

namespace gsi { namespace hipk {

namespace {
constexpr int T_BS = 256;
constexpr int T_R = 4;
constexpr int T_MAXWG = 4096;
struct Lu3State {
  double u[LW][LW];
  double rp[LW];
};

struct Lu3Step {
  double* Y;
  int64_t ld, m;
  int32_t l, j0;
  int s, w;
  double* pval;
  int64_t* pidx;
  Lu3State* stt;
  int32_t* ipiv;
  int32_t* info;
};
__device__ inline void lu3_step_tail(double best, int32_t besti, const Lu3Step& p) {
// ... 170 lines not shown
#pragma unroll
        for (int cc = 0; cc < 4; ++cc) {
          const double* cb = Y + (int64_t)(jb + c + cc) * ld;
#pragma unroll
          for (int rr = 0; rr < T_R; ++rr) {
            const int64_t i = base + rr * T_BS;
            lv[cc][rr] = (i < m) ? cb[i] : 0.0;
          }
        }
#pragma unroll
        for (int cc = 0; cc < 4; ++cc) {
          double u[LW];
#pragma unroll
          for (int k = 0; k < LW; ++k) u[k] = Us[(c + cc) * LW + k];
#pragma unroll
          for (int rr = 0; rr < T_R; ++rr)
#pragma unroll
            for (int k = 0; k < LW; ++k) a[rr][k] -= lv[cc][rr] * u[k];
        }
      }
#pragma unroll
      for (int k = 0; k < LW; ++k) {
        if (k < w) {
          double* cb = Y + (int64_t)(j0 + k) * ld;
#pragma unroll
          for (int rr = 0; rr < T_R; ++rr) {
            const int64_t i = base + rr * T_BS;
            if (i < m) cb[i] = a[rr][k];
          }
        }
      }
#pragma unroll
      for (int rr = 0; rr < T_R; ++rr) {
        const int64_t i = base + rr * T_BS;
        const double av = fabs(a[rr][0]);
        if (i < m && av > best) { best = av; besti = (int32_t)i; }
      }
    }
  }
  lu3_step_tail(best, besti, p);
}

template <int S1>
__global__ __launch_bounds__(T_BS) void lu3_cand_kernel(Lu3Step p) {
  const double* const Y = p.Y;
  const int64_t ld = p.ld, m = p.m;
  const int32_t j0 = p.j0;
  const Lu3State* const stt = p.stt;
  double u[S1][S1 + 1], rp[S1];
#pragma unroll
  for (int t = 0; t < S1; ++t) {
    rp[t] = stt->rp[t];
#pragma unroll
    for (int k = t + 1; k <= S1; ++k) u[t][k] = stt->u[t][k];
  }
  double best = -1.0;
  int32_t besti = -1;
  const int64_t stride = (int64_t)gridDim.x * (T_BS * T_R);
  for (int64_t base = (int64_t)j0 + S1 + (int64_t)blockIdx.x * (T_BS * T_R) + threadIdx.x; base < m; base += stride) {
    double x[T_R][S1 + 1];
#pragma unroll
    for (int k = 0; k <= S1; ++k) {
      const double* cb = Y + (int64_t)(j0 + k) * ld;
#pragma unroll
      for (int rr = 0; rr < T_R; ++rr) {
        const int64_t i = base + rr * T_BS;
        x[rr][k] = (i < m) ? cb[i] : 0.0;
      }
    }
#pragma unroll
    for (int rr = 0; rr < T_R; ++rr) {
#pragma unroll
      for (int t = 0; t < S1; ++t) {
        const double lt = (rp[t] != 0.0) ? x[rr][t] * rp[t] : x[rr][t];
#pragma unroll
        for (int k = t + 1; k <= S1; ++k) x[rr][k] -= lt * u[t][k];
      }
      const int64_t i = base + rr * T_BS;
      const double av = fabs(x[rr][S1]);
      if (i < m && av > best) { best = av; besti = (int32_t)i; }
    }
  }
  lu3_step_tail(best, besti, p);
}

__global__ __launch_bounds__(T_BS) void lu3_close_kernel(double* __restrict__ Y, int64_t ld, int64_t m, int32_t j0, int w,
                                                         const Lu3State* stt) {
  double u[LW][LW], rp[LW];
#pragma unroll
  for (int t = 0; t < LW; ++t) {
    rp[t] = stt->rp[t];
#pragma unroll
    for (int k = t + 1; k < LW; ++k) u[t][k] = stt->u[t][k];
  }
  const int64_t stride = (int64_t)gridDim.x * (T_BS * T_R);
  for (int64_t base = (int64_t)j0 + w + (int64_t)blockIdx.x * (T_BS * T_R) + threadIdx.x; base < m; base += stride) {
    double x[T_R][LW];
#pragma unroll
    for (int k = 0; k < LW; ++k) {
      const double* cb = Y + (int64_t)(j0 + (k < w ? k : 0)) * ld;
#pragma unroll
      for (int rr = 0; rr < T_R; ++rr) {
        const int64_t i = base + rr * T_BS;
        x[rr][k] = (i < m && k < w) ? cb[i] : 0.0;
      }
    }
#pragma unroll
    for (int rr = 0; rr < T_R; ++rr) {
#pragma unroll
      for (int t = 0; t < LW; ++t) {
        if (t < w) {
          const double lt = (rp[t] != 0.0) ? x[rr][t] * rp[t] : x[rr][t];
          x[rr][t] = lt;
#pragma unroll
          for (int k = t + 1; k < LW; ++k) x[rr][k] -= lt * u[t][k];
        }
      }
    }
#pragma unroll
    for (int k = 0; k < LW; ++k) {
      if (k < w) {
        double* cb = Y + (int64_t)(j0 + k) * ld;
#pragma unroll
        for (int rr = 0; rr < T_R; ++rr) {
          const int64_t i = base + rr * T_BS;
          if (i < m) cb[i] = x[rr][k];
        }
      }
    }
  }
}

static int lu3_grid(int64_t rows) {
  const int64_t per = (int64_t)T_BS * T_R;
  const int64_t g = (rows + per - 1) / per;
  return (int)std::max<int64_t>(1, std::min<int64_t>(g, T_MAXWG));
}
}

size_t lu3_work_bytes(int64_t l) {
  return sizeof(double) * T_MAXWG + sizeof(int64_t) * T_MAXWG + sizeof(Lu3State) + sizeof(double) * (size_t)l * (size_t)l +
         sizeof(int32_t) * (size_t)(l + 4) + 512;
}

void lu3_L(hipStream_t st, double* Y, int64_t m, int64_t l, int64_t ld, void* work, int32_t* info, int32_t** ipiv_out) {
  char* base = (char*)work;
  double* pval = (double*)base; base += sizeof(double) * T_MAXWG;
  int64_t* pidx = (int64_t*)base; base += sizeof(int64_t) * T_MAXWG;
  Lu3State* stt = (Lu3State*)base; base += sizeof(Lu3State);
  double* u12 = (double*)base; base += sizeof(double) * (size_t)l * (size_t)l;
  int32_t* ipiv = (int32_t*)base;
  *ipiv_out = ipiv;
  static const bool fuse = !(getenv("GSI_LU_TALL_NOFUSE") != nullptr);
  lu_blocks(st, Y, ld, m, l, LU2_NB, u12, [&](int64_t jb, int b, int64_t j0, int wd) {
    Lu3Step p{Y, ld, m, (int32_t)l, (int32_t)j0, 0, wd, pval, pidx, stt, ipiv, info};
    const int g = lu3_grid(m - j0);
    if (j0 == jb) hipLaunchKernelGGL((lu3_open_kernel<false, false>), dim3(g), dim3(T_BS), 0, st, (int32_t)jb, p);
    else if (fuse) hipLaunchKernelGGL((lu3_open_kernel<true, true>), dim3(g), dim3(T_BS), 0, st, (int32_t)jb, p);
    else hipLaunchKernelGGL((lu3_open_kernel<true, false>), dim3(g), dim3(T_BS), 0, st, (int32_t)jb, p);
    hipLaunchKernelGGL(lu3_pivot_kernel, dim3(1), dim3(T_BS), 0, st, p, g);
    for (int s1 = 1; s1 < wd; ++s1) {
      p.s = s1;
      const int gc = lu3_grid(m - j0 - s1);
      switch (s1) {
        case 1: hipLaunchKernelGGL(lu3_cand_kernel<1>, dim3(gc), dim3(T_BS), 0, st, p); break;
        case 2: hipLaunchKernelGGL(lu3_cand_kernel<2>, dim3(gc), dim3(T_BS), 0, st, p); break;
        case 3: hipLaunchKernelGGL(lu3_cand_kernel<3>, dim3(gc), dim3(T_BS), 0, st, p); break;
        case 4: hipLaunchKernelGGL(lu3_cand_kernel<4>, dim3(gc), dim3(T_BS), 0, st, p); break;
        case 5: hipLaunchKernelGGL(lu3_cand_kernel<5>, dim3(gc), dim3(T_BS), 0, st, p); break;
        case 6: hipLaunchKernelGGL(lu3_cand_kernel<6>, dim3(gc), dim3(T_BS), 0, st, p); break;
        default: hipLaunchKernelGGL(lu3_cand_kernel<7>, dim3(gc), dim3(T_BS), 0, st, p); break;
      }
      hipLaunchKernelGGL(lu3_pivot_kernel, dim3(1), dim3(T_BS), 0, st, p, gc);
    }
    const bool next_opens = fuse && (j0 + wd < jb + b);
    if (m > j0 + wd && !next_opens)
      hipLaunchKernelGGL(lu3_close_kernel, dim3(lu3_grid(m - j0 - wd)), dim3(T_BS), 0, st, Y, ld, m, (int32_t)j0, wd, stt);
  });
}

}}
```

### include/gsi_hip.h

```cpp
#ifndef GSI_HIP_H
#define GSI_HIP_H

#include <stdint.h>

#ifdef __cplusplus
extern "C" {
#endif

#define GSI_VERSION 100

#define GSI_OK 0
#define GSI_ERR_ARG 1
#define GSI_ERR_NEG_ITERS 2
#define GSI_ERR_SINGULAR 3
#define GSI_ERR_HIP 4
#define GSI_ERR_RCCL 5
#define GSI_ERR_OOM 6
#define GSI_ERR_NOT_POSDEF 7
#define GSI_ERR_INTERNAL 8

typedef struct gsi_ctx gsi_ctx;
typedef struct gsi_op gsi_op;
typedef struct gsi_mat gsi_mat;

int gsi_version(void);
const char* gsi_last_error(void);
const char* gsi_backend_name(void);

int gsi_ctx_create(gsi_ctx** ctx, int device_id);
int gsi_ctx_destroy(gsi_ctx* ctx);
int gsi_ctx_sync(gsi_ctx* ctx);

#define GSI_UNIQUE_ID_BYTES 128
int gsi_comm_unique_id(void* id_out);
int gsi_ctx_comm_init(gsi_ctx* ctx, int nranks, int rank, const void* id);
int gsi_ctx_rank(gsi_ctx* ctx, int* rank, int* nranks);
int gsi_ctx_host_allgather(gsi_ctx* ctx, const double* mine, int64_t count, double* all_out);

int gsi_op_dense(gsi_ctx* ctx, gsi_op** op, const double* A_rows, int64_t m, int64_t n,
                 int64_t lda, int64_t row0, int64_t m_local);

int gsi_op_lowrank(gsi_ctx* ctx, gsi_op** op, const double* samples, int64_t n, int64_t N,
                   int64_t lds, int center, int64_t row0, int64_t n_local);

int gsi_op_lowrank_synthetic(gsi_ctx* ctx, gsi_op** op, int64_t n, int64_t N, uint64_t seed, double decay,
                             int64_t row0, int64_t n_local);
int gsi_op_lowrank_samples(gsi_ctx* ctx, const gsi_op* op, double* samples_out, int64_t ld);

int gsi_fftrf_fields(gsi_ctx* ctx, gsi_mat* fields, int ndims, const int64_t* N, double k0, double dk, double beta,
                     const double* phi, int64_t ldphi, uint64_t seed, int64_t field0);
int gsi_op_lowrank_fftrf(gsi_ctx* ctx, gsi_op** op, int ndims, const int64_t* N, double k0, double dk, double beta,
                         int64_t numfields, uint64_t seed, int64_t row0, int64_t n_local);

int gsi_fftrf_interpolate(gsi_ctx* ctx, gsi_mat* out, const gsi_mat* grid, int ndims, const int64_t* N, const double* points,
                          int64_t m, const double* box, int64_t row0);
int gsi_fftrf_spread(gsi_ctx* ctx, gsi_mat* grid_out, const gsi_mat* in, int ndims, const int64_t* N, const double* points,
                     int64_t m, const double* box, int64_t row0);
int gsi_fftrf_fields_at(gsi_ctx* ctx, gsi_mat* out, int ndims, const int64_t* N, double k0, double dk, double beta,
                        const double* phi, int64_t ldphi, uint64_t seed, int64_t field0, const double* points, int64_t m,
                        const double* box, int64_t row0);
int gsi_op_lowrank_fftrf_at(gsi_ctx* ctx, gsi_op** op, int ndims, const int64_t* N, double k0, double dk, double beta,
                            int64_t numfields, uint64_t seed, const double* points, int64_t m, const double* box,
                            int64_t row0, int64_t m_local);

int gsi_op_dense_gridcov(gsi_ctx* ctx, gsi_op** op, int64_t nx, int64_t ny, double ell,
                         int kind, int64_t row0, int64_t m_local);

int gsi_op_gridcov_implicit(gsi_ctx* ctx, gsi_op** op, int64_t nx, int64_t ny, double ell,
                            int64_t row0, int64_t m_local);

int gsi_op_gridcov_implicit_kind(gsi_ctx* ctx, gsi_op** op, int64_t nx, int64_t ny, double ell, int kind, int64_t row0,
                                 int64_t m_local);
int gsi_op_gridcov_implicit_table(gsi_ctx* ctx, gsi_op** op, int64_t nx, int64_t ny, const double* table, int64_t row0,
                                  int64_t m_local);

int gsi_op_pointcov_implicit(gsi_ctx* ctx, gsi_op** op, const double* points, int64_t n, int d, int kind, double ell,
                             double sigma2, double nugget, int64_t row0, int64_t m_local);

int gsi_op_fft_powerlaw(gsi_ctx* ctx, gsi_op** op, int ndims, const int64_t* N, double beta);
int gsi_op_fft_powerlaw_fftrf(gsi_ctx* ctx, gsi_op** op, int ndims, const int64_t* N, double beta);

int gsi_op_fft_gridcov(gsi_ctx* ctx, gsi_op** op, int ndims, const int64_t* N, int kind,
                       const double* ell , double theta, double sigma2, double nugget);
int gsi_op_fft_gridcov_table(gsi_ctx* ctx, gsi_op** op, int ndims, const int64_t* N,
                             const double* table, const double* table_mirror ,
                             double nugget);

int gsi_op_fft_at(gsi_ctx* ctx, gsi_op** op, const gsi_op* grid_op, const double* points, int64_t m, const double* box);

typedef struct gsi_sampler gsi_sampler;
int gsi_gridcov_sampler_create(gsi_ctx* ctx, gsi_sampler** sampler, int ndims, const int64_t* N, const int64_t* embed,
                               int kind, const double* ell , double theta, double sigma2, double nugget,
                               double neg_tol, double* info );
int gsi_gridcov_sampler_info(const gsi_sampler* sampler, int64_t* M , double* info );
int gsi_gridcov_sampler_spectrum(gsi_ctx* ctx, const gsi_sampler* sampler, double* lam_out);
int gsi_gridcov_sampler_destroy(gsi_sampler* sampler);
int gsi_gridcov_fields(gsi_ctx* ctx, const gsi_sampler* sampler, gsi_mat* fields, const double* eps, int64_t ldeps,
                       uint64_t seed, int64_t field0);
int gsi_op_lowrank_gridcov(gsi_ctx* ctx, gsi_op** op, const gsi_sampler* sampler, int64_t numfields, uint64_t seed,
                           int64_t row0, int64_t n_local);

int gsi_op_destroy(gsi_op* op);
int gsi_op_size(const gsi_op* op, int64_t* m, int64_t* n, int64_t* row0, int64_t* m_local);

int gsi_op_mul(gsi_ctx* ctx, const gsi_op* op, int trans, const double* X, int64_t ldx,
               int64_t l, double* Y, int64_t ldy);

int gsi_rangefinder(gsi_ctx* ctx, const gsi_op* op, const double* Omega, int64_t l,
                    int64_t numiterations, double* Q_out);

int gsi_randsvd(gsi_ctx* ctx, const gsi_op* op, const double* Omega, int64_t K, int64_t p,
                int64_t q, double* Z_out, double* S_out);

int gsi_randsvd_dense_host(gsi_ctx* ctx, const double* A_host, int64_t m, int64_t n, int64_t lda, const double* Omega,
                           int64_t K, int64_t p, int64_t q, double* Z_out, double* S_out, gsi_op** op_out);
int gsi_rangefinder_dense_host(gsi_ctx* ctx, const double* A_host, int64_t m, int64_t n, int64_t lda, const double* Omega,
                               int64_t l, int64_t numiterations, double* Q_out, gsi_op** op_out);

int gsi_eig_nystrom(gsi_ctx* ctx, const gsi_op* op, const double* Q, int64_t j,
                    double* U_out, double* Sigma_out);

typedef void (*gsi_randn_fn)(void* user, double* buf, int64_t count);
int gsi_rangefinder_adaptive(gsi_ctx* ctx, const gsi_op* op, gsi_randn_fn randn, void* user,
                             double epsilon, int64_t r, double* Q_out, int64_t* ncols_out);

int gsi_mat_create(gsi_ctx* ctx, gsi_mat** mat, int64_t rows, int64_t cols);
int gsi_mat_destroy(gsi_mat* mat);
int gsi_mat_upload(gsi_ctx* ctx, gsi_mat* mat, const double* host, int64_t ldh);
int gsi_mat_download(gsi_ctx* ctx, const gsi_mat* mat, double* host, int64_t ldh);
int gsi_mat_randn(gsi_ctx* ctx, gsi_mat* mat, uint64_t seed);
int gsi_op_mul_dev(gsi_ctx* ctx, const gsi_op* op, int trans, const gsi_mat* X, gsi_mat* Y);
int gsi_rangefinder_dev(gsi_ctx* ctx, const gsi_op* op, const gsi_mat* Omega,
                        int64_t numiterations, gsi_mat* Q);
int gsi_randsvd_dev(gsi_ctx* ctx, const gsi_op* op, const gsi_mat* Omega, int64_t K, int64_t p,
                    int64_t q, gsi_mat* Z, gsi_mat* S);

int gsi_randsvd_rows(gsi_ctx* ctx, const gsi_op* op, const gsi_mat* Omega_rows, int64_t K, int64_t p, int64_t q,
                     gsi_mat* Z_rows, gsi_mat* S);

int gsi_lu_L(gsi_ctx* ctx, const double* Y, int64_t m, int64_t l, double* L_out, int32_t* ipiv_out);
int gsi_lu_L_dev(gsi_ctx* ctx, gsi_mat* Y, int32_t* ipiv_out);
int gsi_lu_L_sharded(gsi_ctx* ctx, const double* Y, int64_t m, int64_t l, double* L_out, int32_t* ipiv_out);
int gsi_lu_L_sharded_virtual(gsi_ctx* ctx, const double* Y, int64_t m, int64_t l, int nshards, double* L_out,
                             int32_t* ipiv_out);
int gsi_qr_thinQ(gsi_ctx* ctx, const double* Y, int64_t m, int64_t l, double* Q_out, double* R_out);
int gsi_svd_tall(gsi_ctx* ctx, const double* W, int64_t n, int64_t l, double* V_out, double* S_out);
int gsi_gemm(gsi_ctx* ctx, int trans, int64_t m, int64_t l, int64_t k, double alpha,
             const double* A, int64_t lda, const double* B, int64_t ldb, double* C, int64_t ldc);
int gsi_gemm_view(gsi_ctx* ctx, int form, int trans, int64_t m, int64_t l, int64_t k, double alpha, double beta,
                  const double* A, int64_t lda, int64_t a_off, const double* B, int64_t ldb, int64_t b_off,
                  double* C, int64_t ldc, int64_t c_off, int64_t m_full, int64_t r0, int64_t* plan_out);
int gsi_cq_gram_round(gsi_ctx* ctx, int64_t l, int check, const double* gram, double* R, double* X, int32_t* flag_out,
                      int32_t* series_out, double* norm_out);

int gsi_pcga_params(gsi_ctx* ctx, const double* Z, int64_t n, int64_t K, const double* s,
                    const double* X, double delta, double* out);
int gsi_pcga_update(gsi_ctx* ctx, const double* Z, int64_t n, int64_t K, const double* X,
                    double beta_bar, const double* etas, int64_t nobs, const double* xi_bar,
                    double* s_out);

int gsi_pcga_params_dev(gsi_ctx* ctx, const gsi_mat* basis, int64_t K, const double* s, const double* X,
                        double delta, double* out);
int gsi_pcga_update_dev(gsi_ctx* ctx, const gsi_mat* basis, int64_t K, const double* X, double beta_bar,
                        const double* etas, int64_t nobs, const double* xi_bar, double* s_out);
int gsi_mat_download_col(gsi_ctx* ctx, const gsi_mat* mat, int64_t col, double* host);

int gsi_op_lowrank_solve(gsi_ctx* ctx, const gsi_op* op, const double* b, double* x_out, int64_t* iters_out);

int gsi_op_solve_cg(gsi_ctx* ctx, const gsi_op* op, const double* diag, const gsi_mat* B, gsi_mat* X,
                    double tol, int64_t maxiter, int64_t* info, double* relres, int64_t* iters);
int gsi_op_solve(gsi_ctx* ctx, const gsi_op* op, const double* diag, const double* B, int64_t ldb, int64_t b,
                 double* X, int64_t ldx, double tol, int64_t maxiter, int64_t* info, double* relres, int64_t* iters);
int gsi_mat_axpy(gsi_ctx* ctx, double alpha, const gsi_mat* X, gsi_mat* Y);

typedef struct gsi_precond gsi_precond;
int gsi_precond_lowrank_create(gsi_ctx* ctx, gsi_precond** pc, const gsi_mat* Z, int64_t K, const double* diag, double shift,
                               double* info_out);
int gsi_precond_destroy(gsi_precond* pc);
int gsi_precond_info(const gsi_precond* pc, double* info_out);
int gsi_precond_apply(gsi_ctx* ctx, const gsi_precond* pc, const gsi_mat* R, gsi_mat* Zout);
int gsi_op_solve_pcg(gsi_ctx* ctx, const gsi_op* op, const double* diag, const gsi_precond* pc, const gsi_mat* B, gsi_mat* X,
                     double tol, int64_t maxiter, int64_t* info, double* relres, int64_t* iters);
int gsi_op_solve_pcg_host(gsi_ctx* ctx, const gsi_op* op, const double* diag, const gsi_precond* pc, const double* B,
                          int64_t ldb, int64_t b, double* X, int64_t ldx, double tol, int64_t maxiter, int64_t* info,
                          double* relres, int64_t* iters);

int gsi_op_solve_trace(gsi_ctx* ctx, const gsi_op* op, const double* diag, const gsi_precond* pc, const gsi_mat* B, gsi_mat* X,
                       int64_t nquad, int64_t qmax, double tol, int64_t maxiter, int64_t* info, double* relres, int64_t* iters,
                       double* quad_out);
int gsi_slq_quadrature(gsi_ctx* ctx, const double* alpha, const double* beta, const int64_t* steps, const double* rho0,
                       int64_t qmax, int64_t b, double* out);
int gsi_precond_sample(gsi_ctx* ctx, const gsi_precond* pc, const gsi_mat* G1, const gsi_mat* G2, gsi_mat* Zout);
int gsi_precond_logdet(const gsi_precond* pc, double* logdet_out);

int gsi_op_pivoted_cholesky(gsi_ctx* ctx, const gsi_op* op, int64_t K, double tol, gsi_mat* L, int64_t* piv_out, int64_t* info,
                            double* err_out);
int gsi_mat_principal_factor(gsi_ctx* ctx, const gsi_mat* L, int64_t K, gsi_mat* Z_out, double* s_out);

typedef struct gsi_pcgamat gsi_pcgamat;
int gsi_pcgamat_create(gsi_ctx* ctx, gsi_pcgamat** mat, const double* etas, int64_t nobs, int64_t K, const double* HX,
                       const double* R, int r_is_diag);
int gsi_pcgamat_destroy(gsi_pcgamat* mat);
int gsi_pcgamat_mul(gsi_ctx* ctx, const gsi_pcgamat* mat, const double* x, double* y);
int gsi_pcgamat_lsqr(gsi_ctx* ctx, const gsi_pcgamat* mat, const double* b, double* x_out, int64_t* iters_out);
int gsi_pcgamat_solve(gsi_ctx* ctx, const gsi_pcgamat* mat, const double* b, double* x_out, int64_t* info_out);
int gsi_chol_lower(gsi_ctx* ctx, const double* A, int64_t n, int64_t lda, double* L_out, int64_t* info_out);

typedef struct gsi_basis gsi_basis;
int gsi_basis_create(gsi_ctx* ctx, gsi_basis** basis, const gsi_mat* Z, int64_t K, int precision);
int gsi_basis_destroy(gsi_basis* basis);
int gsi_pcga_params_basis(gsi_ctx* ctx, const gsi_basis* basis, const double* s, const double* X, double delta,
                          double* out);
int gsi_pcga_update_basis(gsi_ctx* ctx, const gsi_basis* basis, const double* X, double beta_bar, const double* etas,
                          int64_t nobs, const double* xi_bar, double* s_out);
int gsi_basis_download_col(gsi_ctx* ctx, const gsi_basis* basis, int64_t col, double* host);

typedef struct gsi_fwd gsi_fwd;
int gsi_fwd_linear_create(gsi_ctx* ctx, gsi_fwd** fwd, int64_t nobs, int64_t n, const int64_t* rowptr ,
                          const int64_t* colidx, const double* vals, const double* weights , int link);
int gsi_fwd_destroy(gsi_fwd* fwd);
int gsi_fwd_info(const gsi_fwd* fwd, int64_t* out, int64_t n_out);
int gsi_fwd_apply(gsi_ctx* ctx, const gsi_fwd* fwd, const double* P, int64_t ldp, int64_t ncols, double* out, int64_t ldo);
int gsi_fwd_apply_dev(gsi_ctx* ctx, const gsi_fwd* fwd, const gsi_mat* P , gsi_mat* out );
int gsi_fwd_adjoint_dev(gsi_ctx* ctx, const gsi_fwd* fwd, const gsi_mat* V , gsi_mat* G );
int gsi_fwd_adjoint_info(const gsi_fwd* fwd, int64_t* out, int64_t n_out);
int gsi_op_fwd_cov(gsi_ctx* ctx, gsi_op** op, const gsi_op* grid_op, const gsi_fwd* fwd);
int gsi_pcga_forward_basis(gsi_ctx* ctx, const gsi_basis* basis, const gsi_fwd* fwd, const double* s, const double* X,
                           double delta, double* results_out );

int gsi_basis_quadform(gsi_ctx* ctx, const gsi_basis* basis, const double* W, int64_t ldw, int64_t ncols, int upper,
                       const double* u, double* a_out, double* q_out, double* t_out, int64_t* info_out);
int gsi_pcgamat_posterior(gsi_ctx* ctx, const gsi_pcgamat* mat, double* W_out, double* u_out, double* gamma_out,
                          int64_t* info_out);
int gsi_pcga_posterior_variance(gsi_ctx* ctx, const gsi_basis* basis, const gsi_pcgamat* mat, const double* X,
                                const double* prior, double* var_out, int64_t* info_out);

int gsi_op_posterior_variance(gsi_ctx* ctx, const gsi_op* op, const double* diag, const double* X, int64_t ldx, int64_t p,
                              int64_t batch, double* var_out, int64_t* info_out);
int gsi_mat_rowdot_acc(gsi_ctx* ctx, const gsi_mat* A, const gsi_mat* B, gsi_mat* acc);

#define GSI_PHASE_GEMM_N 0
#define GSI_PHASE_GEMM_T 1
#define GSI_PHASE_LU 2
#define GSI_PHASE_QR 3
#define GSI_PHASE_SVD 4
#define GSI_PHASE_SMALL_GEMM 5
#define GSI_PHASE_COMM 6
#define GSI_PHASE_OTHER 7
#define GSI_PHASE_COMM_WAIT 8
#define GSI_NUM_PHASES 9
int gsi_ctx_profile(gsi_ctx* ctx, int enable);
int gsi_ctx_phase_reset(gsi_ctx* ctx);
int gsi_ctx_phase_times(gsi_ctx* ctx, double* ms_out ,
                        int64_t* count_out );
int gsi_ctx_counters(gsi_ctx* ctx, int64_t* out4);
#define GSI_PATH_LU_FORM_LAST 0
#define GSI_PATH_LU_SELFTEST_MASK 1
#define GSI_PATH_COLLECTIVES 2
#define GSI_PATH_RANKS_SEEN 3
#define GSI_PATH_LU_TIMEOUTS 4
#define GSI_PATH_LU_TIMEOUTS_RECOVERED 5
#define GSI_PATH_LU_FORM_COUNTS 6
#define GSI_PATH_SVD_CAP_HITS 12
#define GSI_PATH_LOWRANK_TAILS 13
#define GSI_PATH_LOWRANK_POWER_STEPS 14
#define GSI_PATH_LOWRANK_POWER_DECLINES 15
#define GSI_PATH_LOWRANK_SPLIT_LUS 16
#define GSI_PATH_LOWRANK_SPLIT_DECLINES 17
#define GSI_PATH_LOWRANK_TAIL_OVERLAPS 18
#define GSI_PATH_LOWRANK_TAIL_SERIES_ROUNDS 19
#define GSI_PATH_INFO_COUNT 20
int gsi_ctx_path_info(gsi_ctx* ctx, int64_t* out, int64_t n_out);
int gsi_ctx_pinned_copy_rate(gsi_ctx* ctx, int64_t bytes, double* h2d_gbs, double* d2h_gbs);
int gsi_ctx_release_cache(gsi_ctx* ctx);
int gsi_ctx_device_bytes(gsi_ctx* ctx, int64_t* bytes);

#ifdef __cplusplus
}
#endif
#endif
```

Measured before the change: 1763.

## Choose variable LU panel block widths with a cost-model DP and column-major U

Replaces the fixed LU block width with a per-block width schedule chosen by a dynamic program over a pass-count cost model (widths 16/32/48/64), overridable through GSI_LU_SCHEDULE. The U12 storage changes from a per-block packed layout to a single column-major l x l buffer. The left-looking update and urows kernels are rewritten to stream this layout in 64-column units with 16-column remainders. The aim is to cut the number of serialized passes and kernel launches in the panel LU of the randSVD rangefinder. In exchange it adds template instantiations and branchy remainder handling, and the cost model may not match the real cost.

```diff
diff --git a/geostatinversion.jl_amd/_lib.py b/geostatinversion.jl_amd/_lib.py
--- a/geostatinversion.jl_amd/_lib.py
+++ b/geostatinversion.jl_amd/_lib.py
@@ -80,6 +80,7 @@
     "gsi_randsvd_dev": (C.c_int, [c_vp, c_vp, c_vp, c_i64, c_i64, c_i64, c_vp, c_vp]),
     "gsi_randsvd_rows": (C.c_int, [c_vp, c_vp, c_vp, c_i64, c_i64, c_i64, c_vp, c_vp]),
     "gsi_lu_L": (C.c_int, [c_vp, c_dp, c_i64, c_i64, c_dp, C.POINTER(C.c_int32)]),
+    "gsi_lu_schedule": (C.c_int, [c_i64, C.POINTER(C.c_int32), C.POINTER(C.c_int32)]),
     "gsi_lu_L_dev": (C.c_int, [c_vp, c_vp, C.POINTER(C.c_int32)]),
     "gsi_lu_L_sharded": (C.c_int, [c_vp, c_dp, c_i64, c_i64, c_dp, C.POINTER(C.c_int32)]),
     "gsi_lu_L_sharded_virtual": (C.c_int, [c_vp, c_dp, c_i64, c_i64, C.c_int, c_dp, C.POINTER(C.c_int32)]),
diff --git a/geostatinversion.jl_amd/build.py b/geostatinversion.jl_amd/build.py
--- a/geostatinversion.jl_amd/build.py
+++ b/geostatinversion.jl_amd/build.py
@@ -11,7 +11,7 @@
 SOURCES = ["gemm_f64.hip", "gemm_f64_gen1.hip", "syrk_f64.hip", "panel_lu_leaf.hip", "panel_lu_blocks.hip", "panel_lu_streamed.hip", "panel_lu_sharded.hip", "panel_qr.hip", "cholqr.hip", "lowrank_power.hip", "jacobi_svd.hip", "misc.hip", "lsqr_dev.hip", "block_cg.hip", "block_pcg.hip", "block_slq.hip", "pivoted_chol.hip", "pointcov_gemm.hip", "fft_cov.hip", "fft_gridcov_plan.hip", "fftrf_sample.hip", "fftrf_interp.hip", "interp_adjoint.hip", "gridcov_sample.hip","pcga_forward.hip", "fwd_adjoint.hip", "chol_saddle.hip", "posterior_var.hip", "posterior_exact.hip",
            "hip_backend.hip", "hip_backend_products.hip", "hip_backend_sampler.hip", "hip_backend_panels.hip", "hip_backend_lowrank.hip", "hip_backend_pcga.hip",
            "hip_comm.hip", "pipeline.cpp", "solvers.cpp", "pcga.cpp", "api.cpp"]
-HEADERS = ["backend.hpp", "hip_backend.hpp", "hip_backend_impl.hpp", "hip_common.hpp", "panel_lu_dev.hpp", "pipeline.hpp", "solvers.hpp", "pcga.hpp", "lsqr_state.hpp", "cg_state.hpp", "block_cg_host.hpp", "slq_state.hpp", "pchol_state.hpp", "pivoted_chol_host.hpp", "pointcov.hpp", "pointcov_gen.hpp", "host_staging.hpp", "gemm_f64_kernel.inc.hpp", "fft_line.hpp", "jacobi_sched.hpp", "fwd_plan.hpp", "fwd_adjoint_plan.hpp", "fwd_adjoint_host.hpp", "fftrf_points.hpp", "interp_adjoint_plan.hpp", "saddle_host.hpp", "posterior_host.hpp", "posterior_exact_host.hpp", "../../include/gsi_hip.h"]
+HEADERS = ["backend.hpp", "hip_backend.hpp", "hip_backend_impl.hpp", "hip_common.hpp", "panel_lu_dev.hpp", "lu_schedule.hpp", "pipeline.hpp", "solvers.hpp", "pcga.hpp", "lsqr_state.hpp", "cg_state.hpp", "block_cg_host.hpp", "slq_state.hpp", "pchol_state.hpp", "pivoted_chol_host.hpp", "pointcov.hpp", "pointcov_gen.hpp", "host_staging.hpp", "gemm_f64_kernel.inc.hpp", "fft_line.hpp", "jacobi_sched.hpp", "fwd_plan.hpp", "fwd_adjoint_plan.hpp", "fwd_adjoint_host.hpp", "fftrf_points.hpp", "interp_adjoint_plan.hpp", "saddle_host.hpp", "posterior_host.hpp", "posterior_exact_host.hpp", "../../include/gsi_hip.h"]
 CXXFLAGS = ["-O3", "-std=c++17", "-fPIC", "--offload-arch=gfx950", "-Wall", "-Wno-unused-function",
             "-Wno-unused-result", "-Wno-unused-value"]
 RESOURCE_FLAG = "-Rpass-analysis=kernel-resource-usage"
diff --git a/geostatinversion.jl_amd/csrc/api.cpp b/geostatinversion.jl_amd/csrc/api.cpp
--- a/geostatinversion.jl_amd/csrc/api.cpp
+++ b/geostatinversion.jl_amd/csrc/api.cpp
@@ -11,6 +11,7 @@
 #include "pointcov.hpp"
 #include "fftrf_points.hpp"
 #include "cg_state.hpp"
+#include "lu_schedule.hpp"
 
 using namespace gsi;
 
@@ -1085,6 +1086,17 @@
   });
 }
 
+int gsi_lu_schedule(int64_t l, int32_t* widths, int32_t* nblocks) {
+  return guarded([&] {
+    REQUIRE(widths && nblocks, "NULL argument");
+    REQUIRE(l >= 1, "lu_schedule: need l >= 1");
+    std::vector<int> w;
+    REQUIRE(lu_schedule_choose(l, w), "lu_schedule: GSI_LU_SCHEDULE is not a list of block widths (16, 32, 48, 64; a last block of 1 .. 64)");
+    for (size_t i = 0; i < w.size(); ++i) widths[i] = w[i];
+    *nblocks = (int32_t)w.size();
+  });
+}
+
 int gsi_lu_L_dev(gsi_ctx* ctx, gsi_mat* Y, int32_t* ipiv_out) {
   return guarded([&] {
     REQUIRE(ctx && Y, "NULL argument");
diff --git a/geostatinversion.jl_amd/csrc/hip_backend_panels.hip b/geostatinversion.jl_amd/csrc/hip_backend_panels.hip
--- a/geostatinversion.jl_amd/csrc/hip_backend_panels.hip
+++ b/geostatinversion.jl_amd/csrc/hip_backend_panels.hip
@@ -1,6 +1,7 @@
 #include <algorithm>
 #include <cstdlib>
 #include "hip_backend_impl.hpp"
+#include "lu_schedule.hpp"
 
 namespace gsi {
 
@@ -30,8 +31,7 @@
     if (const char* e = getenv("GSI_LU_POLL_LIMIT")) w2.poll_limit = atoi(e);
     if (const char* e = getenv("GSI_LU_TEST_MUTE_EPOCH")) w2.mute_epoch = (uint32_t)atoi(e);
     if (const char* e = getenv("GSI_LU_COOPERATIVE")) w2.cooperative = (e[0] == '1');
-    static const int nb_env = getenv("GSI_LU_NB") ? atoi(getenv("GSI_LU_NB")) : 0;
-    w2.nb = (nb_env == 32 || nb_env == 64) ? nb_env : hipk::LU2_NB;
+    if (!lu_schedule_choose(l, w2.widths)) throw Error(GSI_ERR_ARG, "lu: GSI_LU_SCHEDULE is not a list of block widths (16, 32, 48, 64; a last block of 1 .. 64)");
     grow(ws_lu_, hipk::lu2_work_bytes(l, w2.grid));
     hipk::lu2_carve(w2, l, ws_lu_.p);
     w2.info = flags_ + FLAG_LU_INFO;
diff --git a/geostatinversion.jl_amd/csrc/hip_common.hpp b/geostatinversion.jl_amd/csrc/hip_common.hpp
--- a/geostatinversion.jl_amd/csrc/hip_common.hpp
+++ b/geostatinversion.jl_amd/csrc/hip_common.hpp
@@ -3,6 +3,7 @@
 #include <atomic>
 #include <cstdint>
 #include <cstddef>
+#include <vector>
 #include "pointcov.hpp"
 
 namespace gsi { struct FwdProduct; struct FwdAdjoint; }
@@ -112,7 +113,8 @@
   double* u12;
   int32_t* ipiv;
   int32_t* info;
-  int bs, rpt, grid, nb;
+  int bs, rpt, grid;
+  std::vector<int> widths;
   int poll_limit = 0;
   uint32_t mute_epoch = 0;
   bool cooperative = false;
diff --git a/geostatinversion.jl_amd/csrc/lu_schedule.hpp b/geostatinversion.jl_amd/csrc/lu_schedule.hpp
--- /dev/null
+++ b/geostatinversion.jl_amd/csrc/lu_schedule.hpp
@@ -0,0 +1,111 @@
+#pragma once
+#include <cstdint>
+#include <cstdlib>
+#include <cstring>
+#include <vector>
+
+namespace gsi {
+
+constexpr int LU_SCHED_MAX_W = 64;
+constexpr int LU_SCHED_TILE = 16;
+
+constexpr int LU_BLOCK_PASSES = 6;
+
+inline int64_t lu_inblock_passes(int s) {
+  const int64_t nl = (s + 7) / 8;
+  return 4 * nl * (nl - 1);
+}
+inline int64_t lu_block_passes(int64_t jb, int s) {
+  return lu_inblock_passes(s) + (jb > 0 ? jb + 2 * (int64_t)s + LU_BLOCK_PASSES : 0);
+}
+inline int64_t lu_schedule_passes(const std::vector<int>& w) {
+  int64_t jb = 0, sum = 0;
+  for (int s : w) { sum += lu_block_passes(jb, s); jb += s; }
+  return sum;
+}
+inline bool lu_schedule_valid(int64_t l, const std::vector<int>& w) {
+  int64_t sum = 0;
+  for (size_t i = 0; i < w.size(); ++i) {
+    if (w[i] < 1 || w[i] > LU_SCHED_MAX_W) return false;
+    if (i + 1 < w.size() && w[i] % LU_SCHED_TILE != 0) return false;
+    sum += w[i];
+  }
+  return !w.empty() && sum == l;
+}
+inline void lu_schedule_uniform(int64_t l, int nb, std::vector<int>& out) {
+  out.clear();
+  for (int64_t jb = 0; jb < l; jb += nb) out.push_back((int)((l - jb < nb) ? (l - jb) : nb));
+}
+inline void lu_schedule_model(int64_t l, std::vector<int>& out) {
+  out.clear();
+  if (l < 1) return;
+  const int64_t T = (l - 1) / LU_SCHED_TILE;
+  std::vector<int64_t> g((size_t)T + 1);
+  auto step = [&](int64_t t, int s) -> int64_t {
+    const int64_t jb = t * LU_SCHED_TILE, end = jb + s;
+    if (end > l) return -1;
+    if (end == l) return lu_block_passes(jb, s);
+    if (s % LU_SCHED_TILE != 0) return -1;
+    return lu_block_passes(jb, s) + g[(size_t)(end / LU_SCHED_TILE)];
+  };
+  auto widths = [&](int64_t t, int (&w)[5]) -> int {
+    const int64_t left = l - t * LU_SCHED_TILE;
+    int n = 0;
+    for (int s = LU_SCHED_TILE; s <= LU_SCHED_MAX_W && s <= left; s += LU_SCHED_TILE) w[n++] = s;
+    if (left <= LU_SCHED_MAX_W && left % LU_SCHED_TILE != 0) {
+      int i = n++;
+      for (; i > 0 && w[i - 1] > left; --i) w[i] = w[i - 1];
+      w[i] = (int)left;
+    }
+    return n;
+  };
+  for (int64_t t = T; t >= 0; --t) {
+    int w[5];
+    const int n = widths(t, w);
+    int64_t best = -1;
+    for (int i = 0; i < n; ++i) {
+      const int64_t c = step(t, w[i]);
+      if (c >= 0 && (best < 0 || c < best)) best = c;
+    }
+    g[(size_t)t] = best;
+  }
+  for (int64_t t = 0; t * LU_SCHED_TILE < l;) {
+    int w[5];
+    const int n = widths(t, w);
+    for (int i = 0; i < n; ++i)
+      if (step(t, w[i]) == g[(size_t)t]) {
+        out.push_back(w[i]);
+        t = (t * LU_SCHED_TILE + w[i] + LU_SCHED_TILE - 1) / LU_SCHED_TILE;
+        break;
+      }
+  }
+}
+inline bool lu_schedule_parse(const char* s, std::vector<int>& out) {
+  out.clear();
+  while (*s) {
+    char* end = nullptr;
+    const long v = strtol(s, &end, 10);
+    if (end == s || v < 1 || v > 1 << 20) return false;
+    out.push_back((int)v);
+    s = end;
+    if (*s == ',') { ++s; if (!*s) return false; }
+    else if (*s) return false;
+  }
+  return !out.empty();
+}
+inline bool lu_schedule_choose(int64_t l, std::vector<int>& out) {
+  if (const char* e = getenv("GSI_LU_SCHEDULE")) {
+    std::vector<int> w;
+    if (!lu_schedule_parse(e, w)) return false;
+    int64_t sum = 0;
+    for (int s : w) sum += s;
+    if (!lu_schedule_valid(sum, w)) return false;
+    if (sum == l) { out = w; return true; }
+  }
+  const int nb = getenv("GSI_LU_NB") ? atoi(getenv("GSI_LU_NB")) : 0;
+  if (nb == 32 || nb == 64) lu_schedule_uniform(l, nb, out);
+  else lu_schedule_model(l, out);
+  return true;
+}
+
+}
diff --git a/geostatinversion.jl_amd/csrc/panel_lu_blocks.hip b/geostatinversion.jl_amd/csrc/panel_lu_blocks.hip
--- a/geostatinversion.jl_amd/csrc/panel_lu_blocks.hip
+++ b/geostatinversion.jl_amd/csrc/panel_lu_blocks.hip
@@ -24,7 +24,7 @@
 
 template <int K>
 __global__ __launch_bounds__(256) void lu_u12_kernel(const double* __restrict__ Y, int64_t ld, int64_t jb, int64_t jbrow,
-                                                     int64_t c0, int64_t c1, double* __restrict__ out) {
+                                                     int64_t c0, int64_t c1, double* __restrict__ out, int64_t ldo) {
   __shared__ double L11[K * K];
   u12_stage_L11<K>(L11, Y, ld, jb, jbrow);
   __syncthreads();
@@ -36,7 +36,7 @@
 #pragma unroll
   for (int r = 0; r < K; ++r) x[r] = col[r];
   u12_solve<K>(L11, x);
-  double* o = out + (c - c0) * K;
+  double* o = out + (c - c0) * ldo;
 #pragma unroll
   for (int r = 0; r < K; ++r) o[r] = x[r];
 }
@@ -135,9 +135,10 @@
 
 constexpr int LL_WAVES = 12;
 constexpr int LL_BS = 64 * LL_WAVES;
-constexpr size_t LL_LDS = (size_t)4 * 64 * 66 * sizeof(double);
-template <int NB>
-constexpr int ll_group() { return (int)(LL_LDS / ((size_t)NB * (NB + 2) * sizeof(double))); }
+constexpr int LL_UNIT = 64;
+constexpr int LL_KP = LL_UNIT + 2;
+constexpr int LL_GROUP = 4;
+constexpr size_t LL_LDS = (size_t)LL_GROUP * 64 * LL_KP * sizeof(double);
 
 __device__ __forceinline__ char* ll_advance(char* p, int64_t step) {
   p += step;
@@ -147,18 +148,19 @@
 
 template <int NB, bool WIDE>
 __global__ __launch_bounds__(LL_BS) void lu_leftlook_kernel(double* __restrict__ Y, int64_t ld, int64_t m, int64_t jb, int tc,
-                                                            int ip0, int ip1, const double* __restrict__ U12, int64_t ldu) {
+                                                            int p0, int p1, const double* __restrict__ U, int64_t ldu) {
   typedef double double4_t __attribute__((ext_vector_type(4)));
   typedef typename std::conditional<WIDE, uint64_t, uint32_t>::type off_t;
-  constexpr int KP = NB + 2, NT = NB / 16, NS = NB / 4;
+  constexpr int KP = LL_KP, NT = NB / 16, NS = LL_UNIT / 4;
+  typedef std::integral_constant<int, NS> whole_t;
   extern __shared__ double us[];
   const int tid = threadIdx.x, lane = tid & 63;
   const int wave = __builtin_amdgcn_readfirstlane(tid >> 6);
   const int jl = lane & 15, kk = lane >> 4;
-  const int nbk = ip1 - ip0;
-  for (int e = tid; e < nbk * NB * NB; e += LL_BS) {
-    const int k = e % NB, c = (e / NB) % NB, q = e / (NB * NB);
-    us[(q * NB + c) * KP + k] = (c < tc) ? -U12[(int64_t)(ip0 + q) * ldu + (jb + c) * NB + k] : 0.0;
+  const int np = p1 - p0, nfull = np / LL_UNIT, rem = np % LL_UNIT;
+  for (int c = wave; c < NB; c += LL_WAVES) {
+    const double* ucol = U + p0 + (jb + c) * ldu;
+    for (int k = lane; k < np; k += 64) us[((k / LL_UNIT) * NB + c) * KP + k % LL_UNIT] = (c < tc) ? -ucol[k] : 0.0;
   }
   __syncthreads();
   const int lb = jl * KP + kk;
@@ -182,31 +184,48 @@
         }
     }
     double fa[NS], fn[NS];
-    char* pf = reinterpret_cast<char*>(Y + rb + (int64_t)ip0 * NB * ld);
-    auto load_frag = [&](double (&f)[NS]) {
-#pragma unroll
-      for (int s = 0; s < NS; ++s) {
+    char* pf = reinterpret_cast<char*>(Y + rb + (int64_t)p0 * ld);
+    auto load_frag = [&](auto n, double (&f)[NS]) {
+#pragma unroll
+      for (int s = 0; s < decltype(n)::value; ++s) {
         f[s] = *at(pf);
         pf = ll_advance(pf, 4 * cs);
       }
     };
-    auto run = [&](const double (&f)[NS], int q) {
-      const double* ub = us + (q - ip0) * NB * KP + lb;
-#pragma unroll
-      for (int s = 0; s < NS; ++s)
+    auto run = [&](auto n, const double (&f)[NS], int u) {
+      const double* ub = us + u * NB * KP + lb;
+#pragma unroll
+      for (int s = 0; s < decltype(n)::value; ++s)
 #pragma unroll
         for (int tt = 0; tt < NT; ++tt)
           acc[tt] = __builtin_amdgcn_mfma_f64_16x16x4f64(ub[16 * tt * KP + 4 * s], f[s], acc[tt], 0, 0, 0);
     };
-    load_frag(fa);
-    int q = ip0;
-    for (; q + 1 < ip1; ++q) {
-      load_frag(fn);
-      run(fa, q);
-#pragma unroll
-      for (int s = 0; s < NS; ++s) fa[s] = fn[s];
-    }
-    run(fa, q);
+    auto load_rest = [&](double (&f)[NS]) {
+      if (rem == 16) load_frag(std::integral_constant<int, 4>{}, f);
+      else if (rem == 32) load_frag(std::integral_constant<int, 8>{}, f);
+      else if (rem == 48) load_frag(std::integral_constant<int, 12>{}, f);
+    };
+    auto run_rest = [&](const double (&f)[NS]) {
+      if (rem == 16) run(std::integral_constant<int, 4>{}, f, nfull);
+      else if (rem == 32) run(std::integral_constant<int, 8>{}, f, nfull);
+      else if (rem == 48) run(std::integral_constant<int, 12>{}, f, nfull);
+    };
+    if (nfull > 0) {
+      load_frag(whole_t{}, fa);
+      int u = 0;
+      for (; u + 1 < nfull; ++u) {
+        load_frag(whole_t{}, fn);
+        run(whole_t{}, fa, u);
+#pragma unroll
+        for (int s = 0; s < NS; ++s) fa[s] = fn[s];
+      }
+      load_rest(fn);
+      run(whole_t{}, fa, u);
+      run_rest(fn);
+    } else {
+      load_rest(fa);
+      run_rest(fa);
+    }
     const bool live = rb + jl < m;
     char* p = cbase;
 #pragma unroll
@@ -220,9 +239,8 @@
 }
 
 template <int K>
-__global__ __launch_bounds__(256) void lu_urows_kernel(const double* __restrict__ Y, int64_t ld, int64_t jb, int nprev,
-                                                       int64_t c0, int64_t c1, const double* __restrict__ U12, int64_t ldu,
-                                                       double* __restrict__ out) {
+__global__ __launch_bounds__(256) void lu_urows_kernel(const double* __restrict__ Y, int64_t ld, int64_t jb, int64_t c0,
+                                                       int64_t c1, double* U, int64_t ldu) {
   typedef double double4_t __attribute__((ext_vector_type(4)));
   constexpr int TP = K + 1;
   __shared__ double L11[K * K];
@@ -241,15 +259,15 @@
         const int64_t c = cb + 16 * tt + kk + 4 * reg;
         acc[tt][reg] = (c < c1) ? Y[row + c * ld] : 0.0;
       }
-    for (int q = 0; q < nprev; ++q) {
-      const double* ub = U12 + (int64_t)q * ldu;
-#pragma unroll
-      for (int s = 0; s < K / 4; ++s) {
-        const double fa = Y[row + ((int64_t)q * K + 4 * s + kk) * ld];
+    for (int64_t p = 0; p < jb; p += 16) {
+#pragma unroll
+      for (int s = 0; s < 4; ++s) {
+        const int64_t k = p + 4 * s + kk;
+        const double fa = Y[row + k * ld];
 #pragma unroll
         for (int tt = 0; tt < 4; ++tt) {
           const int64_t c = cb + 16 * tt + jl;
-          const double fb = (c < c1) ? -ub[c * K + 4 * s + kk] : 0.0;
+          const double fb = (c < c1) ? -U[k + c * ldu] : 0.0;
           acc[tt] = __builtin_amdgcn_mfma_f64_16x16x4f64(fb, fa, acc[tt], 0, 0, 0);
         }
       }
@@ -267,26 +285,32 @@
 #pragma unroll
   for (int r = 0; r < K; ++r) x[r] = T[tid * TP + r];
   u12_solve<K>(L11, x);
-  double* o = out + (c - c0) * K;
+  double* o = U + jb + c * ldu;
 #pragma unroll
   for (int r = 0; r < K; ++r) o[r] = x[r];
+}
+
+template <class F>
+static void lu_for_width(int w, F&& f) {
+  if (w <= 16) f(std::integral_constant<int, 16>{});
+  else if (w <= 32) f(std::integral_constant<int, 32>{});
+  else if (w <= 48) f(std::integral_constant<int, 48>{});
+  else f(std::integral_constant<int, 64>{});
 }
 
 template <int NB, bool WIDE>
 static void launch_leftlook_v(hipStream_t st, unsigned grid, double* Y, int64_t ld, int64_t m, int64_t jb, int tc,
-                              const double* U12, int64_t ldu) {
+                              const double* U, int64_t ldu) {
   static std::atomic<uint64_t> attr_mask{0};
   if (first_use_on_this_device(attr_mask))
     (void)hipFuncSetAttribute((const void*)lu_leftlook_kernel<NB, WIDE>, hipFuncAttributeMaxDynamicSharedMemorySize, (int)LL_LDS);
-  const int nprev = (int)(jb / NB);
-  for (int ip0 = 0; ip0 < nprev; ip0 += ll_group<NB>()) {
-    const int ip1 = std::min(nprev, ip0 + ll_group<NB>());
-    const size_t shmem = (size_t)(ip1 - ip0) * NB * (NB + 2) * sizeof(double);
-    hipLaunchKernelGGL((lu_leftlook_kernel<NB, WIDE>), dim3(grid), dim3(LL_BS), shmem, st, Y, ld, m, jb, tc, ip0, ip1, U12, ldu);
-  }
-}
-static void lu_ll_update(hipStream_t st, double* Y, int64_t ld, int64_t m, int64_t l, int64_t jb, int b, int nb,
-                         const double* u12) {
+  for (int64_t p0 = 0; p0 < jb; p0 += LL_GROUP * LL_UNIT) {
+    const int64_t p1 = std::min<int64_t>(jb, p0 + LL_GROUP * LL_UNIT);
+    const size_t shmem = (size_t)((p1 - p0 + LL_UNIT - 1) / LL_UNIT) * NB * LL_KP * sizeof(double);
+    hipLaunchKernelGGL((lu_leftlook_kernel<NB, WIDE>), dim3(grid), dim3(LL_BS), shmem, st, Y, ld, m, jb, tc, (int)p0, (int)p1, U, ldu);
+  }
+}
+static void lu_ll_update(hipStream_t st, double* Y, int64_t ld, int64_t m, int64_t l, int64_t jb, int b, const double* u12) {
   if (jb == 0 || m <= jb) return;
   int dev = 0, ncu = 0;
   (void)hipGetDevice(&dev);
@@ -294,27 +318,21 @@
   const int64_t chunks = (m - jb + 15) / 16;
   const unsigned grid = (unsigned)std::min<int64_t>((chunks + LL_WAVES - 1) / LL_WAVES, ncu);
   const bool wide = (3 * ld + 32) * (int64_t)sizeof(double) >= ((int64_t)1 << 32);
-  const int64_t ldu = (int64_t)nb * l;
-  if (nb == 64) {
-    if (wide) launch_leftlook_v<64, true>(st, grid, Y, ld, m, jb, b, u12, ldu);
-    else launch_leftlook_v<64, false>(st, grid, Y, ld, m, jb, b, u12, ldu);
-  } else {
-    if (wide) launch_leftlook_v<32, true>(st, grid, Y, ld, m, jb, b, u12, ldu);
-    else launch_leftlook_v<32, false>(st, grid, Y, ld, m, jb, b, u12, ldu);
-  }
-}
-static void lu_ll_urows(hipStream_t st, const double* Y, int64_t ld, int64_t l, int64_t jb, int nb, double* u12) {
-  const int64_t c0 = jb + nb, ldu = (int64_t)nb * l;
+  lu_for_width(b, [&](auto w) {
+    constexpr int NB = decltype(w)::value;
+    if (wide) launch_leftlook_v<NB, true>(st, grid, Y, ld, m, jb, b, u12, l);
+    else launch_leftlook_v<NB, false>(st, grid, Y, ld, m, jb, b, u12, l);
+  });
+}
+static void lu_ll_urows(hipStream_t st, const double* Y, int64_t ld, int64_t l, int64_t jb, int b, double* u12) {
+  const int64_t c0 = jb + b;
   if (c0 >= l) return;
   const unsigned gu = (unsigned)((l - c0 + 63) / 64);
-  double* out = u12 + (jb / nb) * ldu + c0 * nb;
-  if (nb == 64) {
-    if (jb == 0) hipLaunchKernelGGL(lu_u12_kernel<64>, dim3(gu), dim3(256), 0, st, Y, ld, jb, jb, c0, l, out);
-    else hipLaunchKernelGGL(lu_urows_kernel<64>, dim3(gu), dim3(256), 0, st, Y, ld, jb, (int)(jb / nb), c0, l, u12, ldu, out);
-  } else {
-    if (jb == 0) hipLaunchKernelGGL(lu_u12_kernel<32>, dim3(gu), dim3(256), 0, st, Y, ld, jb, jb, c0, l, out);
-    else hipLaunchKernelGGL(lu_urows_kernel<32>, dim3(gu), dim3(256), 0, st, Y, ld, jb, (int)(jb / nb), c0, l, u12, ldu, out);
-  }
+  lu_for_width(b, [&](auto w) {
+    constexpr int K = decltype(w)::value;
+    if (jb == 0) hipLaunchKernelGGL(lu_u12_kernel<K>, dim3(gu), dim3(256), 0, st, Y, ld, jb, jb, c0, l, u12 + c0 * l, l);
+    else hipLaunchKernelGGL(lu_urows_kernel<K>, dim3(gu), dim3(256), 0, st, Y, ld, jb, c0, l, u12, l);
+  });
 }
 
 __global__ void lu2_extract_L_kernel(double* __restrict__ Y, int64_t ld, int64_t l) {
@@ -326,12 +344,15 @@
   }
 }
 
-void lu_blocks(hipStream_t st, double* Y, int64_t ld, int64_t m, int64_t l, int nb, double* u12, const LuLeafFn& leaf) {
-  for (int64_t jb = 0; jb < l; jb += nb) {
-    const int b = (int)((l - jb < nb) ? (l - jb) : nb);
-    lu_ll_update(st, Y, ld, m, l, jb, b, nb, u12);
+void lu_blocks(hipStream_t st, double* Y, int64_t ld, int64_t m, int64_t l, const std::vector<int>& widths, double* u12,
+               const LuLeafFn& leaf) {
+  if (!lu_schedule_valid(l, widths)) throw std::runtime_error("lu_blocks: the block widths do not fit the panel");
+  int64_t jb = 0;
+  for (const int b : widths) {
+    lu_ll_update(st, Y, ld, m, l, jb, b, u12);
     for (int64_t j0 = jb; j0 < jb + b; j0 += LW) leaf(jb, b, j0, (int)((jb + b - j0 < LW) ? (jb + b - j0) : LW));
-    lu_ll_urows(st, Y, ld, l, jb, nb, u12);
+    lu_ll_urows(st, Y, ld, l, jb, b, u12);
+    jb += b;
   }
   int eb = (int)((l * l + 255) / 256);
   if (eb > 1024) eb = 1024;
@@ -341,8 +362,8 @@
 void lus_u12_block(hipStream_t st, const double* Y, int64_t ld, int64_t row0, int64_t jb, int b, int64_t c0, int64_t c1,
                    double* U12) {
   const unsigned gu = (unsigned)((c1 - c0 + 63) / 64);
-  if (b == 64) hipLaunchKernelGGL(lu_u12_kernel<64>, dim3(gu), dim3(256), 0, st, Y, ld, jb, jb - row0, c0, c1, U12);
-  else hipLaunchKernelGGL(lu_u12_kernel<32>, dim3(gu), dim3(256), 0, st, Y, ld, jb, jb - row0, c0, c1, U12);
+  if (b == 64) hipLaunchKernelGGL(lu_u12_kernel<64>, dim3(gu), dim3(256), 0, st, Y, ld, jb, jb - row0, c0, c1, U12, (int64_t)64);
+  else hipLaunchKernelGGL(lu_u12_kernel<32>, dim3(gu), dim3(256), 0, st, Y, ld, jb, jb - row0, c0, c1, U12, (int64_t)32);
 }
 void lus_rankk(hipStream_t st, double* Y, int64_t ld, int64_t mloc, int64_t row0, int64_t jb, int b, int64_t c0, int64_t t,
                const double* U12) {
diff --git a/geostatinversion.jl_amd/csrc/panel_lu_dev.hpp b/geostatinversion.jl_amd/csrc/panel_lu_dev.hpp
--- a/geostatinversion.jl_amd/csrc/panel_lu_dev.hpp
+++ b/geostatinversion.jl_amd/csrc/panel_lu_dev.hpp
@@ -1,8 +1,11 @@
 #pragma once
 #include "hip_common.hpp"
+#include "lu_schedule.hpp"
 #include <algorithm>
 #include <cstdlib>
 #include <functional>
+#include <stdexcept>
+#include <vector>
 
 namespace gsi { namespace hipk {
 
@@ -87,6 +90,7 @@
 };
 
 using LuLeafFn = std::function<void(int64_t jb, int b, int64_t j0, int wd)>;
-void lu_blocks(hipStream_t st, double* Y, int64_t ld, int64_t m, int64_t l, int nb, double* u12, const LuLeafFn& leaf);
+void lu_blocks(hipStream_t st, double* Y, int64_t ld, int64_t m, int64_t l, const std::vector<int>& widths, double* u12,
+               const LuLeafFn& leaf);
 
 }}
diff --git a/geostatinversion.jl_amd/csrc/panel_lu_leaf.hip b/geostatinversion.jl_amd/csrc/panel_lu_leaf.hip
--- a/geostatinversion.jl_amd/csrc/panel_lu_leaf.hip
+++ b/geostatinversion.jl_amd/csrc/panel_lu_leaf.hip
@@ -817,7 +817,7 @@
 void lu2_L(hipStream_t st, double* Y, int64_t m, int64_t l, int64_t ld, const Lu2Work& w) {
   (void)hipMemsetAsync(w.recs, 0, lu2_record_bytes(w.grid), st);
   uint32_t epoch = 0;
-  lu_blocks(st, Y, ld, m, l, w.nb, w.u12, [&](int64_t jb, int, int64_t j0, int wd) {
+  lu_blocks(st, Y, ld, m, l, w.widths, w.u12, [&](int64_t jb, int, int64_t j0, int wd) {
     if (w.bs == 256 && w.rpt == 1) launch_leaf<256, 1>(st, w.grid, Y, ld, m, l, jb, j0, wd, w, epoch);
     else if (w.bs == 256) launch_leaf<256, 4>(st, w.grid, Y, ld, m, l, jb, j0, wd, w, epoch);
     else if (w.rpt == 4) launch_leaf<512, 4>(st, w.grid, Y, ld, m, l, jb, j0, wd, w, epoch);
diff --git a/geostatinversion.jl_amd/csrc/panel_lu_streamed.hip b/geostatinversion.jl_amd/csrc/panel_lu_streamed.hip
--- a/geostatinversion.jl_amd/csrc/panel_lu_streamed.hip
+++ b/geostatinversion.jl_amd/csrc/panel_lu_streamed.hip
@@ -346,7 +346,9 @@
   int32_t* ipiv = (int32_t*)base;
   *ipiv_out = ipiv;
   static const bool fuse = !(getenv("GSI_LU_TALL_NOFUSE") != nullptr);
-  lu_blocks(st, Y, ld, m, l, LU2_NB, u12, [&](int64_t jb, int b, int64_t j0, int wd) {
+  std::vector<int> widths;
+  lu_schedule_uniform(l, LU2_NB, widths);
+  lu_blocks(st, Y, ld, m, l, widths, u12, [&](int64_t jb, int b, int64_t j0, int wd) {
     Lu3Step p{Y, ld, m, (int32_t)l, (int32_t)j0, 0, wd, pval, pidx, stt, ipiv, info};
     const int g = lu3_grid(m - j0);
     if (j0 == jb) hipLaunchKernelGGL((lu3_open_kernel<false, false>), dim3(g), dim3(T_BS), 0, st, (int32_t)jb, p);
diff --git a/include/gsi_hip.h b/include/gsi_hip.h
--- a/include/gsi_hip.h
+++ b/include/gsi_hip.h
@@ -139,6 +139,7 @@
                      gsi_mat* Z_rows, gsi_mat* S);
 
 int gsi_lu_L(gsi_ctx* ctx, const double* Y, int64_t m, int64_t l, double* L_out, int32_t* ipiv_out);
+int gsi_lu_schedule(int64_t l, int32_t* widths, int32_t* nblocks);
 int gsi_lu_L_dev(gsi_ctx* ctx, gsi_mat* Y, int32_t* ipiv_out);
 int gsi_lu_L_sharded(gsi_ctx* ctx, const double* Y, int64_t m, int64_t l, double* L_out, int32_t* ipiv_out);
 int gsi_lu_L_sharded_virtual(gsi_ctx* ctx, const double* Y, int64_t m, int64_t l, int nshards, double* L_out,
```

Measured after the change: 1790 (median of 6 runs). 1.5% higher.
